# yazinsai/offline-tarteel

Measured on AMD Instinct MI355X. Metric: utterances/sec (10 s @16 kHz), higher is better.
Workload: dtype f16; 1 GPU; c2c-direct-mixed hot path, batch=64/GPU synthetic 10 s/16 kHz clips, FastConformer-CTC forward (fp16 weights) + greedy decode + verse retrieval + CTC rerank (BASELINE.json configs[1]); seeded random weights (real ONNX absent); global_batch=64, parallelism=dp1, gate_failed_utterances_per_batch=64, skip_unused_passes=True, weights=fp16, weights_effective=precision fp16; weights quantised by the engine (none: f16), batches_in_flight=3, concurrent_streams_probe=2

## Files before the change

include/qverse.h:

```cpp
#ifndef QVERSE_H
#define QVERSE_H

#include <stdint.h>

#ifdef __cplusplus
extern "C" {
#endif

#define QV_VOCAB 1025
#define QV_BLANK 1024
#define QV_MAX_TRANSCRIPT 1024
#define QV_MAX_TRANSCRIPT_WIDE 2048

enum {
    QV_OK = 0,
    QV_ERR_ARG = 1,
    QV_ERR_IO = 2,
    QV_ERR_HIP = 3,
    QV_ERR_CAPACITY = 4,
    QV_ERR_NO_MODEL = 5
};

enum { QV_SOURCE_NONE = 0, QV_SOURCE_TEXT = 1, QV_SOURCE_CTC = 2 };

// ... 203 lines not shown
                     qv_align_long_info *info_host, int32_t *first_host, int32_t *last_host, float *logp_host,
                     int32_t pitch, void *stream);
int qv_align_long(qv_engine *e, const float *audio_dev, int64_t audio_pitch, const int64_t *lengths_host, int32_t rows,
                  int32_t window_samples, int32_t margin_frames, const uint16_t *targets_host, const int32_t *lens_host,
                  qv_align_long_info *info_host, int32_t *first_host, int32_t *last_host, float *logp_host,
                  int32_t pitch, void *stream);

#define QV_BEAM_MAX 64
enum { QV_BEAM_COMPLETE = 1 };
typedef struct {
    int32_t node;
    int32_t n_tokens;
    int32_t n_ends;
    int32_t start_verse, span;
    int32_t surah, ayah, ayah_end;
    int32_t below_count;
    int32_t below_verse, below_span;
    int32_t flags;
    double score;
    double blank_score, nonblank_score;
} qv_beam_entry;
typedef struct { int32_t n_entries, t_frames, max_candidates, reserved; } qv_beam_info;

int qv_trie_stats(const char *tables_path, int32_t max_span, int32_t *nodes, int32_t *ends, int32_t *max_depth,
                  int32_t *max_children);
int qv_trie_node_tokens(qv_engine *e, int32_t max_span, int32_t node, int32_t *ids_out, int32_t cap, int32_t *n_out);
int qv_beam_decode(qv_engine *e, const float *logprobs_dev, const int32_t *t_host, int32_t batch, int32_t t_max,
                   int32_t max_span, int32_t beam, int32_t k, qv_beam_info *info_host, qv_beam_entry *entries_host,
                   int32_t *ids_host, int32_t pitch, void *stream);
int qv_beam_batch(qv_engine *e, const float *audio_dev, const int64_t *lengths_host, int32_t batch, int64_t n_max,
                  int32_t max_span, int32_t beam, int32_t k, qv_beam_info *info_host, qv_beam_entry *entries_host,
                  int32_t *ids_host, int32_t pitch, void *stream);

#define QV_SCAN_MAX 32
typedef struct {
    int32_t start_verse, span;
    int32_t surah, ayah, ayah_end;
    int32_t n_tokens;
    float loss, norm;
    double final_score;
} qv_scan_entry;
typedef struct { int32_t n_entries, n_feasible, n_recursions, t_frames; } qv_scan_info;

int qv_scan_stats(const char *tables_path, int32_t t_frames, int32_t max_span, const uint32_t *surah_mask4, int32_t *n_feasible,
                  int32_t *n_recursions, int64_t *state_steps);
int qv_scan_logprobs(qv_engine *e, const float *logprobs_dev, const int32_t *t_host, int32_t batch, int32_t t_max,
                     int32_t max_span, double span_penalty, int32_t k, const uint32_t *surah_mask_host,
                     qv_scan_info *info_host, qv_scan_entry *entries_host, float *loss_out_dev, void *stream);
int qv_scan_batch(qv_engine *e, const float *audio_dev, const int64_t *lengths_host, int32_t batch, int64_t n_max,
                  int32_t max_span, double span_penalty, int32_t k, const uint32_t *surah_mask_host,
                  qv_scan_info *info_host, qv_scan_entry *entries_host, float *loss_out_dev, void *stream);
int qv_scan_kernel_times(qv_engine *e, float *ms2_host);

const int32_t *qv_packed_results_dev(qv_engine *e);


int qv_debug_retrieve(qv_engine *e, const uint8_t *codes_host, int32_t n_codes,
                      int32_t *base_start, int32_t *base_span, double *base_score,
                      int32_t *cand_start, int32_t *cand_span, double *cand_score,
                      int32_t cand_cap, int32_t *n_cand, int32_t *runner_idx, double *runner_score,
                      int32_t *n_runners, void *stream);

int qv_debug_ctc_loss(qv_engine *e, const float *logprobs_dev, int32_t t_frames,
                      const uint16_t *targets_host, const int32_t *lens_host, int32_t n,
                      float *loss_host, void *stream);

int qv_debug_transcript_codes(qv_engine *e, int32_t ctx, int32_t batch, uint8_t *codes_host, int32_t pitch,
                              int32_t *len_host, int32_t *words_host);

int qv_debug_forward_tap(qv_engine *e, int32_t what, int32_t layer, float *out_dev, void *stream);

int qv_profile_gemm(qv_engine *e, int32_t enable);
int qv_profile_gemm_read(qv_engine *e, double *ms21, double *flops21, int32_t *launches21);
int qv_profile_replay_gemm(qv_engine *e, int32_t which, int32_t iters, double *avg_us, double *flops_per_launch,
                           void *stream);
int qv_profile_replay_kernel(qv_engine *e, int32_t which, char *name_out, int32_t name_cap);
int qv_debug_gemm_tiles(int32_t mode);
int qv_debug_gemm_tile_height(int32_t mode);
int qv_debug_gemm_pipeline(int32_t ld, int32_t nst, int32_t narrow);
int qv_debug_attention_variant(int32_t mode);

int qv_debug_kernel_variant(int32_t which, int32_t mode);

int qv_debug_sub01_plan(int64_t n_samples, int32_t batch, int32_t *frames_out, int32_t *run_tiles_out);
int qv_debug_sub35_plan(int64_t n_samples, int32_t batch, int32_t *run_frames_out);

int qv_debug_forward_graph_stats(qv_engine *eng, int64_t *replays, int64_t *captures);
int64_t qv_debug_forward_graph_failures(qv_engine *eng);

int qv_profile_inject_logprobs(qv_engine *e, const float *logprobs_dev, int32_t t_max, const int32_t *t_host, int32_t batch);

int qv_profile_stages(qv_engine *e, int32_t enable);
int qv_stage_times(qv_engine *e, int32_t ctx, float *ms4_host);
int qv_long_kernel_times(qv_engine *e, float *ms3_host);
int qv_align_long_kernel_times(qv_engine *e, float *ms2_host);

int qv_debug_int4_roundtrip(const float *w, int32_t n_rows, int32_t k, float *out);
int qv_debug_int8_roundtrip(const float *w, int32_t n_rows, int32_t k, float *out);

int32_t qv_weight_count(void);
int qv_weight_spec(int32_t index, char *name_out, int32_t name_cap, int32_t *dims4_out, int32_t *ndim_out);
int qv_weight_random(uint64_t seed, int32_t index, float *out, int64_t numel);

int qv_weights_info(qv_engine *e, char *out, int32_t cap);

const char *qv_build_info(void);

#ifdef __cplusplus
}
#endif
#endif
```

offline-tarteel_amd/csrc/qv_capi.hip:

```cpp

#include "qv_common.h"
#include "qv_kernels.h"
#include "qv_layers.h"
#include "qv_long_plan.h"
#include "qv_rows.h"
#include "qv_scan_plan.h"
#include "qv_tables_host.h"
#include "qv_trie_host.h"

#include <math.h>
#include <stdio.h>
#include <string.h>

#include <algorithm>
#include <chrono>
#include <mutex>

static std::string g_create_error;

namespace {
__global__ void k_spin(long long ticks) {
    const long long t0 = wall_clock64();
    while (wall_clock64() - t0 < ticks) __builtin_amdgcn_s_sleep(16);
}
// ... 420 lines not shown
    if (!eng) return QV_ERR_ARG;
    if (enable)
        for (int k = 0; k < eng->n_ctx; ++k)
            for (hipEvent_t &e : eng->ctx[k].stage_ev)
                if (!e) QV_HIP(hipEventCreate(&e));
    eng->profile_stages = enable != 0;
    return QV_OK;
}

extern "C" int qv_stage_times(qv_engine *eng, int32_t k, float *ms4) {
    QV_SERIALISE(eng);
    if (!eng || !ms4 || k < 0 || k >= eng->n_ctx) return QV_ERR_ARG;
    QvCtx &c = eng->ctx[k];
    if (!c.stage_valid) { qv_set_error(eng, "qv_stage_times: no profiled batch on this context (qv_profile_stages first)"); return QV_ERR_ARG; }
    QV_HIP(hipEventSynchronize(c.stage_ev[4]));
    for (int i = 0; i < 4; ++i) QV_HIP(hipEventElapsedTime(&ms4[i], c.stage_ev[i], c.stage_ev[i + 1]));
    return QV_OK;
}

static int fetch_results(qv_engine *eng, QvCtx &c, int batch, int t_max, qv_result *res, int32_t *greedy_host, hipStream_t stream) {
    if (!res || batch < 1 || batch > c.work.max_batch) return QV_ERR_ARG;
    QV_HIP(hipMemcpyAsync(res, c.work.results, sizeof(qv_result) * batch, hipMemcpyDeviceToHost, stream));
    if (greedy_host) {
        int tc = c.work.t_cap;
        int w = t_max < tc ? t_max : tc;
        QV_HIP(hipMemcpy2DAsync(greedy_host, sizeof(int32_t) * t_max, c.work.greedy, sizeof(int32_t) * tc,
                                sizeof(int32_t) * w, batch, hipMemcpyDeviceToHost, stream));
    }
    QV_HIP(hipStreamSynchronize(stream));
    for (int b = 0; b < batch; ++b) {
        if (res[b].source == QV_SOURCE_CTC) res[b].score = exp(-(double)res[b].ctc_norm_loss);
        if (res[b].flags & QV_FLAG_TRANSCRIPT_TRUNCATED) { res[b].surah = res[b].ayah = res[b].ayah_end = 0; }
    }
    return QV_OK;
}

extern "C" int qv_fetch_results(qv_engine *eng, int32_t batch, int32_t t_max, qv_result *res, int32_t *greedy_host,
                                void *stream) {
    QV_SERIALISE(eng);
    if (!eng) return QV_ERR_ARG;
    QV_ORDERED(eng, stream);
    return fetch_results(eng, eng->ctx[eng->cur_ctx], batch, t_max, res, greedy_host, (hipStream_t)stream);
}

extern "C" int qv_decode_retrieve_rerank(qv_engine *eng, const float *lp, const int32_t *t_host, int32_t batch,
                                         int32_t t_max, qv_result *res, int32_t *greedy_host, void *stream) {
    QV_SERIALISE(eng);
    int rc = qv_decode_retrieve_rerank_async(eng, lp, t_host, batch, t_max, stream);
    if (rc) return rc;
    return qv_fetch_results(eng, batch, t_max, res, greedy_host, stream);
}

extern "C" int qv_predict_batch_async(qv_engine *eng, const float *audio_dev, const int64_t *lengths_host,
                                      int32_t batch, int64_t n_max, void *stream) {
    QV_SERIALISE(eng);
    if (!eng) return QV_ERR_ARG;
    QV_TRY(need_model(eng));
    int t_max;
    QV_TRY(batch_in_capacity(eng, "", lengths_host, batch, &t_max));
    QV_ORDERED(eng, stream);
    std::vector<int32_t> t_out(batch);
    hipStream_t run = (hipStream_t)stream;
    if (eng->n_ctx > 1) {
        const int k = eng->next_ctx;
        eng->next_ctx = (k + 1) % eng->n_ctx;
        QvCtx &c = eng->ctx[k];
        if (c.busy) QV_HIP(hipEventSynchronize(c.done));
        eng->cur_ctx = k;
        QV_HIP(hipEventRecord(c.in_ready, (hipStream_t)stream));
        QV_HIP(hipStreamWaitEvent(c.stream, c.in_ready, 0));
        run = c.stream;
    }
    QvCtx &c = eng->ctx[eng->cur_ctx];
    qv_stage_mark(eng, c, 0, run);
    int rc = qv_model_forward(eng, eng->model, eng->cur_ctx, audio_dev, lengths_host, batch, n_max, c.logprobs_ws, t_max,
                              t_out.data(), run, false, eng->n_ctx > 1);
    if (rc) return rc;
    qv_stage_mark(eng, c, 1, run);
    if (eng->inject_lp) {
        if (batch > eng->inject_batch) { qv_set_error(eng, "injected log-probs hold fewer utterances than the batch"); return QV_ERR_ARG; }
        rc = qv_post_run(eng, c, eng->inject_lp, eng->inject_tmax, eng->inject_t.data(), batch, run);
        if (rc == QV_OK) align_note(c, eng->inject_lp, eng->inject_tmax, batch, run);
    } else {
        rc = qv_post_run(eng, c, c.logprobs_ws, t_max, t_out.data(), batch, run);
        if (rc == QV_OK) align_note(c, c.logprobs_ws, t_max, batch, run);
    }
    if (rc) return rc;
    if (eng->n_ctx > 1) {
        QV_HIP(hipEventRecord(c.done, c.stream));
        c.busy = true;
    }
    return QV_OK;
}

extern "C" int qv_predict_batch_async_ctx(qv_engine *eng, const float *audio_dev, const int64_t *lengths_host, int32_t batch,
                                          int64_t n_max, void *stream, int32_t *ctx_out) {
    QV_SERIALISE(eng);
    int rc = qv_predict_batch_async(eng, audio_dev, lengths_host, batch, n_max, stream);
    if (rc == QV_OK && ctx_out) *ctx_out = eng->cur_ctx;
    return rc;
}

extern "C" int qv_predict_batch(qv_engine *eng, const float *audio_dev, const int64_t *lengths_host, int32_t batch,
                                int64_t n_max, qv_result *res, int32_t *greedy_host, void *stream) {
    QV_SERIALISE(eng);
    int rc = qv_predict_batch_async(eng, audio_dev, lengths_host, batch, n_max, stream);
    if (rc) return rc;
    const int last_tmax = eng->ctx[eng->cur_ctx].last_tmax;
    if (eng->n_ctx > 1) return qv_fetch_results_ctx(eng, eng->cur_ctx, batch, last_tmax, res, greedy_host);
    return qv_fetch_results(eng, batch, last_tmax, res, greedy_host, stream);
}

static int fir_for(qv_engine *eng, const float *taps, int32_t n_taps, int32_t up, const qv_engine::Fir **out);

extern "C" int qv_upfirdn(qv_engine *eng, const float *x_dev, int64_t n_in, const float *taps, int32_t n_taps, int32_t up,
                          int32_t down, int64_t m0, int64_t n_out, float *y_dev, void *stream) {
    QV_SERIALISE(eng);
    if (!eng || !x_dev || !taps || !y_dev || n_in < 1 || n_taps < 1 || up < 1 || down < 1 || m0 < 0 || n_out < 0) return QV_ERR_ARG;
    QV_ORDERED(eng, stream);
    const qv_engine::Fir *fir = nullptr;
    QV_TRY(fir_for(eng, taps, n_taps, up, &fir));
    launch_upfirdn(x_dev, n_in, fir->hflip_dev, fir->P, up, down, m0, n_out, y_dev, (hipStream_t)stream);
    QV_HIP(hipGetLastError());
    return QV_OK;
}

static int fir_for(qv_engine *eng, const float *taps, int32_t n_taps, int32_t up, const qv_engine::Fir **out) {
    for (const auto &f : eng->firs)
        if (f.up == up && (int)f.taps.size() == n_taps && memcmp(f.taps.data(), taps, sizeof(float) * n_taps) == 0) { *out = &f; return QV_OK; }
    int P = (n_taps + up - 1) / up;
    std::vector<float> hf((size_t)up * P, 0.f);
    for (int t = 0; t < up; ++t)
        for (int j = 0; j < P; ++j) {
            int k = t + up * (P - 1 - j);
            if (k < n_taps) hf[(size_t)t * P + j] = taps[k];
        }
    float *d = nullptr;
    QV_TRY(qv_dev_zeroed(eng, eng->allocs, hf.size(), &d));
    QV_HIP(hipMemcpy(d, hf.data(), hf.size() * sizeof(float), hipMemcpyHostToDevice));
    eng->firs.push_back({up, std::vector<float>(taps, taps + n_taps), d, P});
    *out = &eng->firs.back();
    return QV_OK;
}

static int resample_slot(qv_engine *eng, unsigned char **slot) {
    if (!eng->resample_tab) QV_TRY(qv_dev_zeroed(eng, eng->allocs, (size_t)QV_RESAMPLE_SLOTS * QV_RESAMPLE_ROWS * 12, &eng->resample_tab));
    *slot = eng->resample_tab + (size_t)(eng->resample_at++ % QV_RESAMPLE_SLOTS) * QV_RESAMPLE_ROWS * 12;
    return QV_OK;
}

extern "C" int qv_upfirdn_batch(qv_engine *eng, const float *x_dev, int64_t x_pitch, const int32_t *src_rows_host,
                                const int64_t *n_in_host, int32_t rows, const float *taps, int32_t n_taps, int32_t up, int32_t down,
                                int64_t m0, float *y_dev, int64_t y_pitch, void *stream) {
    QV_SERIALISE(eng);
    if (!eng || !x_dev || !n_in_host || !taps || !y_dev || rows < 1 || rows > QV_RESAMPLE_ROWS || n_taps < 1 || up < 1 || down < 1 || m0 < 0 ||
        x_pitch < 1 || y_pitch < 1)
        return QV_ERR_ARG;
    for (int r = 0; r < rows; ++r) {
        if (n_in_host[r] < 1 || n_in_host[r] > x_pitch) { qv_set_error(eng, "qv_upfirdn_batch: a row's length is outside [1, x_pitch]"); return QV_ERR_ARG; }
        if ((n_in_host[r] * up + down - 1) / down > y_pitch) { qv_set_error(eng, "qv_upfirdn_batch: y_pitch is shorter than a row's output"); return QV_ERR_ARG; }
        if (src_rows_host && src_rows_host[r] < 0) return QV_ERR_ARG;
    }
    QV_ORDERED(eng, stream);
    const qv_engine::Fir *fir = nullptr;
    QV_TRY(fir_for(eng, taps, n_taps, up, &fir));
    unsigned char *slot = nullptr;
    QV_TRY(resample_slot(eng, &slot));
// ... 540 lines not shown
    memcpy(ms3_host, eng->long_ws.kernel_ms, sizeof(float) * 3);
    return QV_OK;
}

extern "C" int qv_align_long_kernel_times(qv_engine *eng, float *ms2_host) {
    QV_SERIALISE(eng);
    if (!eng || !ms2_host) return QV_ERR_ARG;
    if (!eng->profile_stages || !eng->align_long_ws.big) { qv_set_error(eng, "qv_align_long_kernel_times: no profiled long alignment (qv_profile_stages first)"); return QV_ERR_ARG; }
    memcpy(ms2_host, eng->align_long_ws.kernel_ms, sizeof(float) * 2);
    return QV_OK;
}

extern "C" int qv_debug_forward_tap(qv_engine *eng, int32_t what, int32_t layer, float *out_dev, void *stream) {
    QV_SERIALISE(eng);
    if (!eng) return QV_ERR_ARG;
    if (!eng->model) { qv_set_error(eng, "engine created without a model"); return QV_ERR_NO_MODEL; }
    QV_ORDERED(eng, stream);
    return qv_model_tap(eng, eng->model, eng->cur_ctx, what, layer, out_dev, (hipStream_t)stream);
}

extern "C" int qv_profile_gemm(qv_engine *eng, int32_t enable) {
    if (!eng) return QV_ERR_ARG;
    qv_gemm_prof_enable(enable != 0);
    return QV_OK;
}

extern "C" int qv_profile_gemm_read(qv_engine *eng, double *ms21, double *flops21, int32_t *launches21) {
    if (!eng || !ms21 || !flops21 || !launches21) return QV_ERR_ARG;
    int n[21];
    qv_gemm_prof_collect(ms21, flops21, n);
    for (int i = 0; i < 21; ++i) launches21[i] = n[i];
    return QV_OK;
}

extern "C" int qv_profile_replay_kernel(qv_engine *eng, int32_t which, char *name_out, int32_t name_cap) {
    QV_SERIALISE(eng);
    if (!eng || !name_out || name_cap < 8) return QV_ERR_ARG;
    if (!eng->model) { qv_set_error(eng, "engine created without a model"); return QV_ERR_NO_MODEL; }
    return qv_model_replay_kernel(eng, eng->model, eng->cur_ctx, which, name_out, name_cap);
}

extern "C" int qv_weights_info(qv_engine *eng, char *out, int32_t cap) {
    QV_SERIALISE(eng);
    if (!eng || !out || cap < 16) return QV_ERR_ARG;
    if (!eng->model) { snprintf(out, (size_t)cap, "no acoustic model (post-logits stages only)"); return QV_OK; }
    qv_model_weights_info(eng->model, out, cap);
    return QV_OK;
}

extern "C" int qv_debug_attention_variant(int32_t mode) {
    if (mode < -1 || mode > 5) return QV_ERR_ARG;
    qv_attention_set_variant(mode);
    return QV_OK;
}

extern "C" int qv_debug_kernel_variant(int32_t which, int32_t mode) {
    if (which < 0 || which >= QV_KV_COUNT || mode < -1 || mode > 15) return QV_ERR_ARG;
    qv_kernel_variant_set(which, mode);
    return QV_OK;
}

extern "C" int qv_debug_sub01_plan(int64_t n_samples, int32_t batch, int32_t *frames_out, int32_t *run_tiles_out) {
    if (n_samples < 400 || batch < 1 || !frames_out) return QV_ERR_ARG;
    qv_model_frame_counts(n_samples, frames_out);
    if (run_tiles_out) *run_tiles_out = qv_sub01_run_tiles(batch, frames_out[2], qv_switches_now());
    return QV_OK;
}

extern "C" int qv_debug_sub35_plan(int64_t n_samples, int32_t batch, int32_t *run_frames_out) {
    if (n_samples < 400 || batch < 1 || !run_frames_out) return QV_ERR_ARG;
    int32_t fr[4];
    qv_model_frame_counts(n_samples, fr);
    *run_frames_out = qv_sub35_run_frames(batch, fr[3], qv_switches_now());
    return QV_OK;
}

extern "C" int qv_debug_forward_graph_stats(qv_engine *eng, int64_t *replays, int64_t *captures) {
    QV_SERIALISE(eng);
    if (!eng || !eng->model || !replays || !captures) return QV_ERR_ARG;
    qv_model_graph_stats(eng->model, replays, captures);
    return QV_OK;
}

extern "C" int64_t qv_debug_forward_graph_failures(qv_engine *eng) {
    QV_SERIALISE(eng);
    return (eng && eng->model) ? qv_model_graph_failures(eng->model) : -1;
}

extern "C" int qv_debug_gemm_tiles(int32_t mode) {
    if (mode < -1 || mode > 2) return QV_ERR_ARG;
    qv_gemm_set_t256(mode);
    return QV_OK;
}

extern "C" int qv_debug_gemm_tile_height(int32_t mode) {
    if (mode < -1 || mode > 3) return QV_ERR_ARG;
    qv_gemm_set_bm(mode);
    return QV_OK;
}

extern "C" int qv_debug_gemm_pipeline(int32_t ld, int32_t nst, int32_t narrow) {
    const int ids[3] = {QV_SW_GEMM_LD, QV_SW_GEMM_NST, QV_SW_GEMM_NARROW}, modes[3] = {ld, nst, narrow};
    for (int i = 0; i < 3; ++i)
        if (modes[i] < -1 || modes[i] > QV_SWITCH_TABLE[ids[i]].hi) return QV_ERR_ARG;
    for (int i = 0; i < 3; ++i) qv_switch_set(ids[i], modes[i]);
    return QV_OK;
}

extern "C" int qv_profile_replay_gemm(qv_engine *eng, int32_t which, int32_t iters, double *avg_us, double *flops_per_launch,
                                      void *stream) {
    QV_SERIALISE(eng);
    if (!eng || !avg_us || !flops_per_launch) return QV_ERR_ARG;
    if (!eng->model) { qv_set_error(eng, "engine created without a model"); return QV_ERR_NO_MODEL; }
    return qv_model_replay_gemm(eng, eng->model, eng->cur_ctx, which, iters, avg_us, flops_per_launch, (hipStream_t)stream);
}
```

offline-tarteel_amd/csrc/qv_common.h:

```cpp
#pragma once

#include <hip/hip_runtime.h>
#include <stdint.h>

#include <algorithm>
#include <functional>
#include <mutex>
#include <string>
#include <vector>

#include "../../include/qverse.h"
#include "qv_limits.h"
#include "qv_long_plan.h"
#include "qv_switches.h"

#define QV_CAND_CAP 2048
#define QV_RUNNER_CAP 128
#define QV_RAW_CAP 4096

#define QV_HIP(expr)                                                                         \
    do {                                                                                     \
        hipError_t e_ = (expr);                                                              \
        if (e_ != hipSuccess) {                                                              \
            qv_set_error(eng, std::string(#expr) + ": " + hipGetErrorString(e_));            \
// ... 188 lines not shown
    QvMirror m;
    size_t row_bytes, ops_cap;
    size_t in_off, bp_off;
    size_t bp_row_words;
};
int qv_correct_rows(qv_engine *eng, QvCtx &c, const uint8_t *pred_codes, const int32_t *pred_off, const uint8_t *ref_codes,
                    const int32_t *ref_off, int rows, int flags, qv_correct_info *info_host, uint8_t *ops_host, int ops_pitch,
                    qv_correct_word *words_host, int words_pitch, hipStream_t stream);
int qv_correct_results(qv_engine *eng, int k_ctx, int batch, int flags, qv_correct_info *info_host, uint8_t *ops_host, int ops_pitch,
                       qv_correct_word *words_host, int words_pitch);

int qv_transcribe_rows(qv_engine *eng, QvCtx &c, const float *lp, const int32_t *t_host, int batch, int t_max,
                       qv_transcript_info *info_host, int32_t *ids_host, float *logp_host, int16_t *first_host, int16_t *last_host,
                       int pitch, hipStream_t stream);

struct QvBeamState;
struct QvTrie;
void qv_beam_free(qv_engine *eng);
int qv_beam_trie(qv_engine *eng, int max_span, const QvTrie **out);
int qv_beam_node_tokens(qv_engine *eng, int max_span, int node, int32_t *ids_out, int cap, int32_t *n_out);
int qv_beam_rows(qv_engine *eng, QvCtx &c, const float *lp, const int32_t *t_host, int batch, int t_max, int max_span, int W, int k,
                 qv_beam_info *info_host, qv_beam_entry *entries_host, int32_t *ids_host, int pitch, hipStream_t stream);

struct QvScanState;
void qv_scan_free(qv_engine *eng);
int qv_scan_times(qv_engine *eng, float *ms2);
int qv_scan_rows(qv_engine *eng, QvCtx &c, const float *lp, const int32_t *t_host, int batch, int t_max, int max_span, double penalty,
                 int k, const uint32_t *mask_host, qv_scan_info *info_host, qv_scan_entry *entries_host, float *loss_out_dev,
                 hipStream_t stream);

struct QvLongWs {
    QvMirror m;
    float *batch;
    size_t batch_cap;
    size_t tab_bytes, rec_bytes, out_bytes, fid_bytes;
    float kernel_ms[3];
};
void qv_long_free(QvLongWs &w);
int qv_long_run(qv_engine *eng, QvCtx &c, const float *audio, int64_t audio_pitch, const float *lp_in, int t_max_in,
                const int64_t *n_host, int rows, int window_samples, int margin_frames, qv_long_info *info_host, int32_t *ids_host,
                float *logp_host, int32_t *first_host, int32_t *last_host, int pitch, hipStream_t stream);
struct QvLongWin {
    int64_t src_off;
    int64_t dst;
    int32_t len;
    int32_t lp_win;
    int32_t j0;
    int32_t count;
};
struct QvLongRec { int32_t t_frames, n_windows; };
struct QvLongTimer;
struct QvLongCall {
    std::vector<QvLongPlan> plans;
    std::vector<int64_t> fwd_len;
    size_t n_win;
    int t_top, kw, wn, P;
    const QvLongWin *tab_d;
    const QvLongRec *rec_d;
};
int qv_long_check(qv_engine *eng, const char *who, QvCtx &c, const float *audio, int64_t audio_pitch, int t_max_in,
                  const int64_t *n_host, int rows, int window_samples, int margin_frames, QvLongCall &call);
int qv_long_tables(qv_engine *eng, QvCtx &c, bool audio, int64_t audio_pitch, int rows, QvLongCall &call, hipStream_t stream);
int qv_long_rounds(qv_engine *eng, QvCtx &c, const QvLongCall &call, const float *audio, int64_t audio_pitch, const float *lp_in,
                   int t_max_in, hipStream_t stream, QvLongTimer *tm,
                   const std::function<int(const float *lp, int t_max, size_t k0, int nb)> &per_round);

struct QvAlignLongWs {
    QvMirror m;
    unsigned char *big;
    size_t big_bytes;
    float kernel_ms[3];
};
void qv_align_long_free(QvAlignLongWs &w);
int qv_align_long_run(qv_engine *eng, QvCtx &c, const float *audio, int64_t audio_pitch, const float *lp_in, int t_max_in,
                      const int64_t *n_host, int rows, int window_samples, int margin_frames, const uint16_t *targets_host,
                      const int32_t *lens_host, qv_align_long_info *info_host, int32_t *first_host, int32_t *last_host,
                      float *logp_host, int pitch, hipStream_t stream);

struct QvMatchSet {
    int max_q;
    int decode_threads;
    int frag_blocks;
    size_t trigram_lds;
    void (*k_decode)(QvTables, QvWork, const float *, int, const int32_t *);
    void (*k_prepare_codes)(QvWork, int);
    void (*k_trigram)(QvTables, QvWork), (*k_frag)(QvTables, QvWork);
    void (*k_lcs_full)(QvTables, QvWork, int), (*k_hint_sp)(QvTables, QvWork, int);
    void (*k_spans)(QvTables, QvWork, QvKnobs), (*k_spans2)(QvTables, QvWork, QvKnobs);
    void (*k_track)(QvTables, QvTrack);
    void (*k_ctc_long[2])(QvTables, QvWork, QvKnobs, const float *, int);
};
extern const QvMatchSet qv_match_default __attribute__((visibility("hidden"))), qv_match_wide __attribute__((visibility("hidden")));

int qv_post_tracker_match(qv_engine *eng, const uint8_t *codes_host, const int32_t *offsets_host,
                          const int32_t *n_words_host, const int32_t *bonus_host, int batch,
                          qv_track_match *out_host, hipStream_t stream);
int qv_post_run(qv_engine *eng, QvCtx &c, const float *logprobs_dev, int t_max, const int32_t *t_host, int batch,
                hipStream_t stream);
int qv_post_debug_retrieve(qv_engine *eng, QvCtx &c, const uint8_t *codes_host, int n, hipStream_t stream);
int qv_post_match_verse(qv_engine *eng, QvCtx &c, const uint8_t *codes_host, int n, int n_bonus, const int32_t *bonus_verse,
                        const double *bonus_value, int max_span, hipStream_t stream);
int qv_post_debug_ctc(qv_engine *eng, const float *lp, int T, const uint16_t *tg, const int32_t *lens, int n,
                      float *loss_host, hipStream_t stream);

struct QvModel;
int qv_model_create(qv_engine *eng, const qv_config *cfg, const QvSwitches &sw, QvModel **out);
void qv_model_destroy(QvModel *m);
int qv_model_forward(qv_engine *eng, QvModel *m, int k, const float *audio_dev, const int64_t *len_host, int batch,
                     int64_t n_max, float *logprobs_dev, int t_max, int32_t *t_out_host, hipStream_t stream,
                     bool zero_pad_rows = false,
                     bool may_graph = false);
int qv_model_tap(qv_engine *eng, QvModel *m, int k, int what, int layer, float *out_dev, hipStream_t stream);
void qv_model_frame_counts(int64_t n_samples, int32_t out[4]);
int qv_model_replay_gemm(qv_engine *eng, QvModel *m, int k, int which, int iters, double *avg_us, double *flops, hipStream_t s);
int qv_model_replay_kernel(qv_engine *eng, QvModel *m, int k, int which, char *name_out, int cap);

void qv_model_weights_info(const QvModel *m, char *out, int cap);
void qv_model_graph_stats(const QvModel *m, int64_t *replays, int64_t *captures);
int64_t qv_model_graph_failures(const QvModel *m);
void qv_stage_mark(qv_engine *eng, QvCtx &c, int i, hipStream_t s);

#define QV_MAX_CTX 8
#define QV_STAGE_SLOTS 2
struct QvCtx {
    QvWork work = {};
    float *logprobs_ws = nullptr;
    int32_t *t_host_scratch = nullptr;
    int32_t *t_dev = nullptr;
    hipStream_t stream = nullptr;
    hipEvent_t in_ready = nullptr, done = nullptr;
    bool busy = false;
    int last_batch = 0, last_tmax = 0;
    hipEvent_t t_copied[QV_STAGE_SLOTS] = {};
    bool t_pending[QV_STAGE_SLOTS] = {};
    int t_slot = 0;
    hipEvent_t stage_ev[5] = {};
    bool stage_valid = false;
    struct PostGraph { const float *lp; int batch, t_max, variants; hipGraphExec_t exec; } post_graph[4] = {};
    bool post_graph_off = false;
    int n_post_graph = 0;
    const float *al_lp = nullptr;
    int al_tmax = 0, al_batch = 0;
    hipStream_t al_stream = nullptr;
    std::vector<QvMirror> mirrors;
    QvAlignWs align = {};
    QvNbestWs nbest = {};
    QvCorrectWs correct = {};
    QvRowWs transcribe = {};
    QvRowWs beam = {};
    QvMirror scan = {};
};

struct qv_engine {
    std::recursive_mutex mu;
    hipEvent_t tail_ev = nullptr;
    hipStream_t tail_stream = nullptr;
    bool tail_valid = false;
    qv_config cfg;
    int max_q = QV_MAX_TRANSCRIPT;
    const QvMatchSet *match = &qv_match_default;
    QvKnobs knobs;
    int device;
    std::string last_error;
    QvTables tab;
    std::vector<void *> allocs;
    QvCtx ctx[QV_MAX_CTX];
    int n_ctx, cur_ctx, next_ctx;
    QvModel *model;
    struct Fir { int up; std::vector<float> taps; float *hflip_dev; int P; };
    std::vector<Fir> firs;
    unsigned char *resample_tab = nullptr;
    unsigned resample_at = 0;
    QvTrack track;
    QvLongWs long_ws = {};
    QvAlignLongWs align_long_ws = {};
    QvBeamState *beam = nullptr;
    QvScanState *scan = nullptr;
    bool profile_stages;
    const float *inject_lp;
    int inject_tmax, inject_batch;
    std::vector<int32_t> inject_t;
    std::vector<uint8_t> h_surah;
    std::vector<uint16_t> h_ayah;
};
```

offline-tarteel_amd/csrc/qv_dev_util.h:

```cpp
#pragma once

#include "qv_kernels.h"

static __device__ __forceinline__ float wave_sum(float v) {
#pragma unroll
    for (int o = 32; o > 0; o >>= 1) v += __shfl_xor(v, o);
    return v;
}
static __device__ __forceinline__ float wave_max(float v) {
#pragma unroll
    for (int o = 32; o > 0; o >>= 1) v = fmaxf(v, __shfl_xor(v, o));
    return v;
}
static __device__ __forceinline__ float wave_min(float v) {
#pragma unroll
    for (int o = 32; o > 0; o >>= 1) v = fminf(v, __shfl_xor(v, o));
    return v;
}

static __device__ __forceinline__ int xcd_order(int wg, int nwg) {
    const int q = nwg >> 3, r = nwg & 7, xcd = wg & 7, idx = wg >> 3;
    return (xcd < r ? xcd * (q + 1) : r * (q + 1) + (xcd - r) * q) + idx;
}

static __device__ __forceinline__ void mel_mean_rstd(const double *acc, int b, int f, int tm, float &mean, float &rstd) {
    double s1 = acc[((size_t)b * QV_NMEL + f) * 2], s2 = acc[((size_t)b * QV_NMEL + f) * 2 + 1];
    double mu = s1 / tm, var = (s2 - s1 * mu) / (tm - 1);
    mean = (float)mu;
    rstd = 1.f / (sqrtf((float)(var > 0.0 ? var : 0.0)) + 1e-5f);
}

struct LnParam { f32x4 g0, g1, b0, b1; };
static __device__ __forceinline__ LnParam ln_param(const float *__restrict__ gam, const float *__restrict__ bet, int lane) {
    LnParam p;
    p.g0 = *(const f32x4 *)(gam + lane * 8); p.g1 = *(const f32x4 *)(gam + lane * 8 + 4);
    p.b0 = *(const f32x4 *)(bet + lane * 8); p.b1 = *(const f32x4 *)(bet + lane * 8 + 4);
    return p;
}
static __device__ __forceinline__ void ln_row_p(const float v[8], const LnParam &p, float o[8]) {
    float s = 0.f;
#pragma unroll
    for (int i = 0; i < 8; ++i) s += v[i];
    float mu = wave_sum(s) * (1.f / QV_D);
    float q = 0.f;
#pragma unroll
    for (int i = 0; i < 8; ++i) { float d = v[i] - mu; q += d * d; }
    float rs = rsqrtf(wave_sum(q) * (1.f / QV_D) + 1e-5f);
#pragma unroll
    for (int i = 0; i < 4; ++i) { o[i] = (v[i] - mu) * rs * p.g0[i] + p.b0[i]; o[4 + i] = (v[4 + i] - mu) * rs * p.g1[i] + p.b1[i]; }
}

static __device__ __forceinline__ void conv0_tap_offsets(int hi, int koff[5]) {
#pragma unroll
    for (int j = 0; j < 5; ++j) {
        const int k = 2 * j + hi < 9 ? 2 * j + hi : 8;
        koff[j] = (k / 3) * (QV_NMEL + 2) + k % 3;
    }
}
static __device__ __forceinline__ void conv0_taps(const float *rows, int r0, int f1, const int koff[5], float xb[5]) {
    const float *base = rows + r0 * (QV_NMEL + 2) + 2 * f1;
#pragma unroll
    for (int j = 0; j < 5; ++j) xb[j] = base[koff[j]];
}
```

offline-tarteel_amd/csrc/qv_launch_plan.h:

```cpp
#pragma once

#include "qv_limits.h"
#include "qv_switches.h"

enum GemmWeights { GEMM_W_F16 = 0, GEMM_W_INT4 = 1, GEMM_W_INT8 = 2, GEMM_W_A8W8 = 3 };
struct GemmShape {
    int M, N, K;
    int weights;
    bool has_bias;
    bool glu;
    int in_flight;
};
struct GemmPlan { bool wide, narrow; int nst, bm; };

inline GemmPlan gemm_plan(const GemmShape &g, const QvSwitches &sw) {
    const bool w4 = g.weights == GEMM_W_INT4;
    const int env_nst = sw[QV_SW_GEMM_NST], env_narrow = sw[QV_SW_GEMM_NARROW], env_ld = sw[QV_SW_GEMM_LD];
    GemmPlan p;
    p.narrow = g.N % 128 != 0;
    if (w4 && !p.narrow && (g.N / 128) * ((g.M + 127) / 128) < 400) p.narrow = true;
    if (env_narrow >= 0 && g.N % 128 == 0 && !g.glu) p.narrow = env_narrow != 0;
    const int tiles = (g.N / (p.narrow ? 64 : 128)) * ((g.M + 127) / 128);
    p.nst = tiles >= 400 ? 2 : (g.K / 64 >= 16 ? 4 : 3);
    if (p.narrow && p.nst > 3) p.nst = 3;
    if (env_nst >= 2 && env_nst <= (p.narrow ? 3 : 4)) p.nst = env_nst;
    if (env_ld == 1) p.nst = 0;
    const int t256 = sw[QV_SW_GEMM_T256];
    p.wide = false;
    p.bm = 256;
    if (t256 > 0 && g.N % 256 == 0 && g.has_bias && !(w4 && (g.K % 128 != 0 || g.K > 4096))) {
        const int tiles256 = (g.N / 256) * ((g.M + 255) / 256);
        const int env_min = sw[QV_SW_GEMM_MINTILES], env_min_longk = sw[QV_SW_GEMM_MINTILES_LONGK];
        const bool busy = g.in_flight >= 3;
        const int min_tiles = env_min > 0 ? env_min : g.in_flight >= 4 ? 1 : busy ? 128 : 160;
        const int min_tiles_longk = env_min_longk > 0 ? env_min_longk : busy ? 1 : 160;
        p.wide = t256 >= 2 || tiles256 >= (g.K >= 2048 ? min_tiles_longk : min_tiles);
        const int bm_mode = sw[QV_SW_GEMM_BM];
        if (p.wide && bm_mode > 0) {
            const long tiles192 = (long)(g.N / 256) * ((g.M + 191) / 192);
            const long cost256 = ((tiles256 + 255) / 256) * 256, cost192 = ((tiles192 + 255) / 256) * 192;
            if (bm_mode >= 3 || ((bm_mode == 2 || !busy) && cost192 * 108 <= cost256 * 100)) p.bm = 192;
        }
    }
    return p;
}

struct GemmKernel { int bn, nst, ld; };
inline GemmKernel gemm_kernel(const GemmShape &g, const GemmPlan &p) {
    if (g.weights == GEMM_W_INT8 || g.weights == GEMM_W_A8W8) return {128, 2, 1};
    const int bn = p.narrow && !g.glu ? 64 : 128;
    if (p.nst == 0) return {bn, 2, 1};
    return {bn, p.nst <= 2 ? 2 : p.nst == 3 || bn == 64 ? 3 : 4, 0};
}

inline int sub01_run_tiles(int batch, int t2_max, const QvSwitches &sw) {
    const int n_tiles = (t2_max + SUB_TT - 1) / SUB_TT, forced = sw[QV_KV_SUB_RUN];
    int best = 1;
    if (forced >= 1 && forced <= 4) best = forced == 3 ? SUB_MAX_RUN : forced == 4 ? SUB_RES_RUN : forced;
    else {
        long best_cost = -1;
        for (int run = 1; run <= SUB_RES_RUN; ++run) {
            const long blocks = (long)batch * ((n_tiles + run - 1) / run), cost = (blocks + 511) / 512 * (2 * run + 1);
            if (best_cost < 0 || cost < best_cost) { best = run; best_cost = cost; }
        }
    }
    return best < n_tiles ? best : (n_tiles > 0 ? n_tiles : 1);
}

inline int sub35_run_steps(int batch, int t3_max, const QvSwitches &sw) {
    const int n_steps = (t3_max + S35_TC - 1) / S35_TC, forced = sw[QV_KV_SUB35];
    int best = 1;
    if (forced >= 1 && forced <= 3) best = forced == 3 ? S35_MAX_RUN : forced;
    else {
        long best_cost = -1;
        for (int run = 1; run <= S35_MAX_RUN; ++run) {
            const long blocks = (long)batch * ((n_steps + run - 1) / run), cost = (blocks + 255) / 256 * (run + 1);
            if (best_cost < 0 || cost < best_cost) { best = run; best_cost = cost; }
        }
    }
    return best < n_steps ? best : (n_steps > 0 ? n_steps : 1);
}

enum AttKernel { ATT_NONE, ATT_WS_2_2_192, ATT_WS_1_3_256, ATT_X_192, ATT_OLD };
struct AttentionPlan {
    bool run_short;
    int rest;
    int t_short;
};
inline AttentionPlan attention_plan(int variant, int t_min, int t_max) {
    if (variant == 2) return {false, ATT_OLD, 0};
    AttentionPlan p = {false, ATT_NONE, 0};
    if (variant == 3 || variant == 5) {
        p.t_short = ATT_SHORT_T;
        p.run_short = t_min <= ATT_SHORT_T;
        if (t_max <= ATT_SHORT_T) return p;
    }
    p.rest = variant == 4 || variant == 5 ? ATT_X_192 : variant == 1 ? ATT_WS_1_3_256 : ATT_WS_2_2_192;
    return p;
}
```

offline-tarteel_amd/csrc/qv_layers.h:

```cpp
#pragma once

#include "qv_kernels.h"

struct FrontendTab {
    const float *window;
    const float2 *twiddle;
    const int32_t *mel_lo;
    const int32_t *mel_cnt;
    const float *mel_w;
};

size_t qv_melstats_doubles(size_t max_batch);
void launch_logmel(const float *audio, int64_t n_max, const int32_t *n_samples, const FrontendTab &ft, float *feats,
                   int tm_max, double *stats, int batch, hipStream_t s, const QvSwitches &sw = qv_switches_now());
void launch_melapply(const float *feats, const int32_t *n_samples, int tm_max, const double *stats, float *out, int batch,
                     hipStream_t s);
void launch_conv0(const float *feats, int tm_max, const int32_t *len_in, const double *stats, const float *w,
                  const float *bias, half_t *out, int t1_max, int batch, hipStream_t s);
void launch_sub01(const float *feats, int tm_max, const int32_t *len_mel, const double *stats, const float *w0,
                  const float *b0, const int32_t *len1, const float *w1, const float *b1, half_t *out, int t2_max, int batch,
                  hipStream_t s, const QvSwitches &sw = qv_switches_now());
int qv_sub01_run_tiles(int batch, int t2_max, const QvSwitches &sw = qv_switches_now());
void launch_dwconv2d(const half_t *in, int tin_max, int fin, const int32_t *len_in, const float *w, const float *bias,
                     half_t *out, int tout_max, int fout, int batch, hipStream_t s);
void launch_pack_rows(const half_t *x, int t_max, int row_elems, const int32_t *len, const int32_t *row_off, half_t *y,
                      int32_t *row_map, int batch, hipStream_t s);
void launch_sub35(const half_t *c1, int t2_max, const half_t *w3, const float *b3, const float *w5, const float *b5,
                  const int32_t *len2, const int32_t *len3, const int32_t *row_off, half_t *out, int32_t *row_map, int t3_max,
                  int batch, hipStream_t s, const QvSwitches &sw = qv_switches_now());
void qv_sub35_init();
int qv_sub35_run_frames(int batch, int t3_max, const QvSwitches &sw = qv_switches_now());
void launch_unpack_rows_f32(const half_t *x, int t_max, int row_elems, const int32_t *len, const int32_t *row_off, float *y,
                            int batch, hipStream_t s);
void launch_layernorm(const float *x, const float *g, const float *b, half_t *y, int M, hipStream_t s);
void launch_layernorm2(float *x, const float *g1, const float *b1, const float *g2, const float *b2, half_t *y, int M,
                       hipStream_t s);
void launch_to_half(const float *x, half_t *y, size_t n, hipStream_t s);
void launch_to_float(const half_t *x, float *y, size_t n, hipStream_t s);
void launch_attention(const half_t *qk, const half_t *vt, const half_t *pos, int pos_ld, const float *bu, const float *bv,
                      const int32_t *len, const int32_t *row_off, half_t *out, int t_max, int t_min, int t_pad, int batch,
                      hipStream_t s, const QvSwitches &sw = qv_switches_now());
void launch_dwconv1d(const half_t *x, const float *w, const float *bias, const int32_t *len, const int32_t *row_off, half_t *y,
                     int t_max, int batch, hipStream_t s);
void launch_logsoftmax(const float *logits, int ld, float *out, int M, const int32_t *row_map, int t_out, hipStream_t s);
void launch_zero_pad_rows(float *out, const int32_t *len, int t_out, int t_min, int batch, hipStream_t s);
void launch_upfirdn_rows(const float *x, int64_t x_pitch, const int32_t *src, const int64_t *n_in_rows, int rows, const float *hflip,
                         int P, int up, int down, int64_t m0, float *y, int64_t y_pitch, hipStream_t s);
void launch_mixdown(const float *x, int64_t x_pitch, const int64_t *n_frames, int rows, int channels, float *y, int64_t y_pitch,
                    int64_t max_frames, hipStream_t s);
void launch_upfirdn(const float *x, int64_t n_in, const float *hflip, int P, int up, int down, int64_t m0, int64_t n_out,
                    float *y, hipStream_t s);
```

offline-tarteel_amd/csrc/qv_layers.hip:

```cpp

#include "qv_layers.h"

#include "qv_dev_util.h"
#include "qv_launch_plan.h"
#include "qv_logmel_reg.h"

#include <math.h>

namespace {

__device__ __forceinline__ float sigmoidf_(float x) { return 1.0f / (1.0f + __expf(-x)); }

__global__ __launch_bounds__(256) void k_logmel(const float *__restrict__ audio, int64_t n_max,
                                                const int32_t *__restrict__ n_samples, const FrontendTab ft,
                                                float *__restrict__ feats, int tm_max) {
    __shared__ float2 buf[4][2][256];
    __shared__ float pw[4][264];
    __shared__ float2 tw[256];
    const int wave = threadIdx.x >> 6, lane = threadIdx.x & 63;
    const int b = blockIdx.y, t = blockIdx.x * 4 + wave;
    const int n = n_samples[b];
    const int tm = n / 160 + 1;
    tw[threadIdx.x] = ft.twiddle[threadIdx.x];
    __syncthreads();
// ... 660 lines not shown
            else {
#pragma unroll
                for (int i = 0; i < 8; ++i) o2[i] = o[i];
            }
            half8 h;
#pragma unroll
            for (int i = 0; i < 8; ++i) h[i] = (half_t)o2[i];
            *(half8 *)(y + (size_t)(row0 + r) * QV_D + lane * 8) = h;
        }
    }
}

__global__ void k_to_half(const float *__restrict__ x, half_t *__restrict__ y, size_t n8) {
    size_t i = (size_t)blockIdx.x * blockDim.x + threadIdx.x;
    if (i >= n8) return;
    f32x4 a = *(const f32x4 *)(x + i * 8), c = *(const f32x4 *)(x + i * 8 + 4);
    half8 h = {(half_t)a[0], (half_t)a[1], (half_t)a[2], (half_t)a[3], (half_t)c[0], (half_t)c[1], (half_t)c[2], (half_t)c[3]};
    *(half8 *)(y + i * 8) = h;
}

__global__ void k_to_float(const half_t *__restrict__ x, float *__restrict__ y, size_t n) {
    size_t i = (size_t)blockIdx.x * blockDim.x + threadIdx.x;
    if (i < n) y[i] = (float)x[i];
}

#define DW_TT 4
__global__ __launch_bounds__(256) void k_dwconv1d(const half_t *__restrict__ x, const float *__restrict__ wt ,
                                                  const float *__restrict__ bias, const int32_t *__restrict__ len,
                                                  const int32_t *__restrict__ row_off, half_t *__restrict__ y) {
    const int wg = xcd_order(blockIdx.y * gridDim.x + blockIdx.x, gridDim.x * gridDim.y);
    const int b = wg / gridDim.x, t0 = ((wg - b * gridDim.x) * 4 + (threadIdx.x >> 6)) * DW_TT, lane = threadIdx.x & 63;
    const int T = len[b], c0 = lane * 8;
    if (t0 >= T) return;
    const size_t row0 = (size_t)row_off[b];
    float w[9][8], bs[8];
#pragma unroll
    for (int k = 0; k < 9; ++k) {
        f32x4 w0 = *(const f32x4 *)(wt + k * QV_D + c0), w1 = *(const f32x4 *)(wt + k * QV_D + c0 + 4);
#pragma unroll
        for (int c = 0; c < 4; ++c) { w[k][c] = w0[c]; w[k][4 + c] = w1[c]; }
    }
    {
        f32x4 b0 = *(const f32x4 *)(bias + c0), b1 = *(const f32x4 *)(bias + c0 + 4);
#pragma unroll
        for (int c = 0; c < 4; ++c) { bs[c] = b0[c]; bs[4 + c] = b1[c]; }
    }
    float acc[DW_TT][8];
#pragma unroll
    for (int j = 0; j < DW_TT; ++j)
#pragma unroll
        for (int c = 0; c < 8; ++c) acc[j][c] = bs[c];
#pragma unroll
    for (int i = 0; i < DW_TT + 8; ++i) {
        int tt = t0 - 4 + i;
        if (tt < 0 || tt >= T) continue;
        half8 v = *(const half8 *)(x + (row0 + tt) * QV_D + c0);
        float vf[8];
#pragma unroll
        for (int c = 0; c < 8; ++c) vf[c] = (float)v[c];
#pragma unroll
        for (int j = 0; j < DW_TT; ++j) {
            int k = i - j;
            if (k < 0 || k > 8) continue;
#pragma unroll
            for (int c = 0; c < 8; ++c) acc[j][c] = __builtin_fmaf(w[k][c], vf[c], acc[j][c]);
        }
    }
#pragma unroll
    for (int j = 0; j < DW_TT; ++j) {
        if (t0 + j >= T) break;
        half8 o;
#pragma unroll
        for (int c = 0; c < 8; ++c) o[c] = (half_t)(acc[j][c] * sigmoidf_(acc[j][c]));
        *(half8 *)(y + (row0 + t0 + j) * QV_D + c0) = o;
    }
}

__global__ __launch_bounds__(256) void k_logsoftmax(const float *__restrict__ logits, int ld, float *__restrict__ out, int M,
                                                    const int32_t *__restrict__ row_map, int t_out) {
    int row = blockIdx.x * 4 + (threadIdx.x >> 6), lane = threadIdx.x & 63;
    if (row >= M) return;
    const int bt = row_map[row];
    const size_t orow = (size_t)(bt >> 16) * t_out + (bt & 0xFFFF);
    const float *p = logits + (size_t)row * ld;
    float v[17];
    float mx = -INFINITY;
#pragma unroll
    for (int i = 0; i < 17; ++i) {
        int c = lane + 64 * i;
        v[i] = c < 1025 ? p[c] : -INFINITY;
        mx = fmaxf(mx, v[i]);
    }
    mx = wave_max(mx);
    float s = 0.f;
#pragma unroll
    for (int i = 0; i < 17; ++i) s += (lane + 64 * i < 1025) ? expf(v[i] - mx) : 0.f;
    float lse = mx + logf(wave_sum(s));
    float *o = out + orow * 1025;
#pragma unroll
    for (int i = 0; i < 17; ++i) {
        int c = lane + 64 * i;
        if (c < 1025) o[c] = v[i] - lse;
    }
}

__global__ __launch_bounds__(256) void k_zero_pad_rows(float *__restrict__ out, const int32_t *__restrict__ len, int t_out) {
    const int b = blockIdx.y, t = len[b] + blockIdx.x;
    if (t >= t_out) return;
    float *o = out + ((size_t)b * t_out + t) * 1025;
    for (int c = threadIdx.x; c < 1025; c += 256) o[c] = 0.f;
}

}


size_t qv_melstats_doubles(size_t max_batch) { return max_batch * 2 * QV_NMEL * (1 + MS_CHUNKS); }

void launch_logmel(const float *audio, int64_t n_max, const int32_t *n_samples, const FrontendTab &ft, float *feats,
                   int tm_max, double *stats, int batch, hipStream_t s, const QvSwitches &sw) {
    double *part = stats + (size_t)batch * 2 * QV_NMEL;
    const int variant = sw[QV_KV_LOGMEL];
    if (variant == 2)
        hipLaunchKernelGGL(lmv::k_logmel_run<QV_LOGMEL_RUN>, dim3((tm_max + 4 * QV_LOGMEL_RUN - 1) / (4 * QV_LOGMEL_RUN), batch), dim3(256), 0, s, audio, n_max, n_samples, ft, feats, tm_max);
    else if (variant == 1)
        hipLaunchKernelGGL(lmv::k_logmel_reg<0>, dim3((tm_max + 3) / 4, batch), dim3(256), 0, s, audio, n_max, n_samples, ft, feats, tm_max);
    else
        hipLaunchKernelGGL(k_logmel, dim3((tm_max + 3) / 4, batch), dim3(256), 0, s, audio, n_max, n_samples, ft, feats, tm_max);
    hipLaunchKernelGGL(k_melstats, dim3(MS_CHUNKS, batch), dim3(320), 0, s, feats, n_samples, tm_max, part);
    hipLaunchKernelGGL(k_melstats_sum, dim3(batch), dim3(2 * QV_NMEL), 0, s, part, stats);
}

void launch_melapply(const float *feats, const int32_t *n_samples, int tm_max, const double *stats, float *out, int batch,
                     hipStream_t s) {
    hipLaunchKernelGGL(k_melapply, dim3(64, batch), dim3(320), 0, s, feats, n_samples, tm_max, stats, out);
}

void launch_conv0(const float *feats, int tm_max, const int32_t *len_in, const double *stats, const float *w,
                  const float *bias, half_t *out, int t1_max, int batch, hipStream_t s) {
    hipLaunchKernelGGL(k_conv0, dim3(1, t1_max, batch), dim3(256), 0, s, feats, tm_max, len_in, stats, w, bias, out, t1_max);
}

int qv_sub01_run_tiles(int batch, int t2_max, const QvSwitches &sw) { return sub01_run_tiles(batch, t2_max, sw); }

void launch_sub01(const float *feats, int tm_max, const int32_t *len_mel, const double *stats, const float *w0,
                  const float *b0, const int32_t *len1, const float *w1, const float *b1, half_t *out, int t2_max, int batch,
                  hipStream_t s, const QvSwitches &sw) {
    const int n_tiles = (t2_max + SUB_TT - 1) / SUB_TT, run = sub01_run_tiles(batch, t2_max, sw);
    const dim3 grid(1, (n_tiles + run - 1) / run, batch);
    if (run <= SUB_RES_RUN)
        hipLaunchKernelGGL(k_sub01<true>, grid, dim3(256), 0, s, feats, tm_max, len_mel, stats, w0, b0, len1, w1, b1, out, t2_max, run);
    else
        hipLaunchKernelGGL(k_sub01<false>, grid, dim3(256), 0, s, feats, tm_max, len_mel, stats, w0, b0, len1, w1, b1, out, t2_max, run);
}

void launch_dwconv2d(const half_t *in, int tin_max, int fin, const int32_t *len_in, const float *w, const float *bias,
                     half_t *out, int tout_max, int fout, int batch, hipStream_t s) {
    hipLaunchKernelGGL(k_dwconv2d, dim3(1, (tout_max + DW2_TT - 1) / DW2_TT, batch), dim3(256), 0, s, in, tin_max, fin, len_in, w,
                       bias, out, tout_max, fout);
}

void launch_pack_rows(const half_t *x, int t_max, int row_elems, const int32_t *len, const int32_t *row_off, half_t *y,
                      int32_t *row_map, int batch, hipStream_t s) {
    hipLaunchKernelGGL(k_pack_rows, dim3(1, t_max, batch), dim3(256), 0, s, x, t_max, row_elems, len, row_off, y, row_map);
}

int qv_sub35_run_frames(int batch, int t3_max, const QvSwitches &sw) { return sub35_run_steps(batch, t3_max, sw) * S35_TC; }

void qv_sub35_init() {
    static const int once = [] {
        (void)hipFuncSetAttribute((const void *)k_sub35, hipFuncAttributeMaxDynamicSharedMemorySize, S35_LDS);
        return 0;
    }();
    (void)once;
}

void launch_sub35(const half_t *c1, int t2_max, const half_t *w3, const float *b3, const float *w5, const float *b5,
                  const int32_t *len2, const int32_t *len3, const int32_t *row_off, half_t *out, int32_t *row_map, int t3_max,
                  int batch, hipStream_t s, const QvSwitches &sw) {
    qv_sub35_init();
    const int n_steps = (t3_max + S35_TC - 1) / S35_TC, run = sub35_run_steps(batch, t3_max, sw);
    hipLaunchKernelGGL(k_sub35, dim3(1, (n_steps + run - 1) / run, batch), dim3(512), S35_LDS, s, c1, t2_max, w3, b3, w5, b5, len2,
                       len3, row_off, out, row_map, run);
}

void launch_unpack_rows_f32(const half_t *x, int t_max, int row_elems, const int32_t *len, const int32_t *row_off, float *y,
// ... 172 lines not shown
```

offline-tarteel_amd/csrc/qv_match_body.inc:

```
#define QV_MAXW (QV_MAXQ / 64)

#include "qv_post_util.h"
#include "qv_lcs.h"
#include <type_traits>

namespace QV_MATCH_NS {

#define DEC_WAVES 16
__global__ __launch_bounds__(64 * DEC_WAVES) void k_decode(QvTables tab, QvWork wk, const float *__restrict__ lp, int t_max,
                                                          const int32_t *__restrict__ t_dev) {
    __shared__ uint8_t raw[QV_RAW_CAP];
    __shared__ unsigned long long pm[2][QV_NSYM][QV_MAXW];
    __shared__ int16_t s_fid[QV_FRAME_CAP];
    __shared__ int32_t s_tok[QV_FRAME_CAP];
    const int b = blockIdx.x, tid = threadIdx.x, lane = tid & 63, wave = tid >> 6;
    if (b == 0 && tid == 0) { *wk.n_fail = 0; wk.frag_ctr[0] = 0; wk.frag_ctr[1] = 0; wk.frag_ctr[2] = 0; }
    QvUtt &u = wk.utt[b];
    const int T = t_dev[b];
    for (int t = wave; t < T; t += DEC_WAVES) {
        float best;
        int bi;
        frame_argmax(lp + ((size_t)b * t_max + t) * QV_VOCAB, lane, best, bi);
        if (lane == 0) s_fid[t] = (int16_t)bi;
    }
    __syncthreads();
    if (wave != 0) return;
    int32_t *greedy = wk.greedy + (size_t)b * wk.t_cap;
    int n_tok = 0;
    for (int base = 0; base < T; base += 64) {
        int t = base + lane;
        int id = -1;
        bool keep = false;
        if (t < T) {
            id = s_fid[t];
            int prev = t > 0 ? s_fid[t - 1] : -1;
            keep = id != prev && id != QV_BLANK;
        }
        int tot, r = wave_rank(keep, lane, tot);
        if (keep) { s_tok[n_tok + r] = id; greedy[n_tok + r] = id; }
        n_tok += tot;
    }
    for (int t = n_tok + lane; t < wk.t_cap; t += 64) greedy[t] = -1;
    QV_WSYNC();
    int n_raw = 0;
    bool trunc = false;
    for (int base = 0; base < n_tok; base += 64) {
        int k = base + lane;
        int id = k < n_tok ? s_tok[k] : -1;
        int len = id >= 0 ? (int)(tab.piece_off[id + 1] - tab.piece_off[id]) : 0;
        int incl = len;
#pragma unroll
        for (int o = 1; o < 64; o <<= 1) {
            int x = __shfl_up(incl, o);
            if (lane >= o) incl += x;
        }
        int off = n_raw + incl - len;
        if (off + len > QV_RAW_CAP) { trunc = true; len = 0; }
        const uint8_t *src = tab.piece_codes + (id >= 0 ? tab.piece_off[id] : 0);
        for (int i = 0; i < len; ++i) raw[off + i] = src[i];
        n_raw += __shfl(incl, 63);
    }
    trunc = __any(trunc);
    if (n_raw > QV_RAW_CAP) n_raw = QV_RAW_CAP;
    QV_WSYNC();
    int last_ns = -1;
    for (int i = lane; i < n_raw; i += 64)
        if (raw[i] != 0) last_ns = i;
    last_ns = wave_max_i(last_ns);
    uint8_t *q = wk.q + (size_t)b * QV_MAXQ, *qs = wk.qs + (size_t)b * QV_MAXQ;
    unsigned long long *pmf = &pm[0][0][0];
    for (int i = lane; i < 2 * QV_NSYM * QV_MAXW; i += 64) pmf[i] = 0ull;
    QV_WSYNC();
    int qn = 0, qsn = 0, spaces = 0;
    for (int base = 0; base < n_raw; base += 64) {
        int i = base + lane;
        int c = i < n_raw ? raw[i] : 0;
        bool keep = i < n_raw && (c != 0 ? true : (i > 0 && raw[i - 1] != 0 && i < last_ns));
        int tot, r = wave_rank(keep, lane, tot);
        if (keep && qn + r < QV_MAXQ) {
            q[qn + r] = (uint8_t)c;
            if (c < QV_NSYM) atomicOr(&pm[0][c][(qn + r) >> 6], 1ull << ((qn + r) & 63));
        }
        bool ks = keep && c != 0;
        int tots, rs = wave_rank(ks, lane, tots);
        if (ks && qsn + rs < QV_MAXQ) {
            qs[qsn + rs] = (uint8_t)c;
            if (c < QV_NSYM) atomicOr(&pm[1][c][(qsn + rs) >> 6], 1ull << ((qsn + rs) & 63));
        }
        spaces += tot - tots;
        qn += tot;
        qsn += tots;
    }
    if (qn > QV_MAXQ) trunc = true;
    int flags = 0;
    if (trunc) { flags |= QV_FLAG_TRANSCRIPT_TRUNCATED; qn = 0; qsn = 0; }
    else if (qn == 0) flags |= QV_FLAG_EMPTY_TRANSCRIPT;
    QV_WSYNC();
    uint64_t *gpm = wk.pm + (size_t)b * 2 * QV_NSYM * QV_MAXW;
    for (int i = lane; i < 2 * QV_NSYM * QV_MAXW; i += 64) gpm[i] = trunc ? 0ull : pmf[i];
    if (lane == 0) {
        u.t_frames = T;
        u.n_tok = n_tok;
        u.q_len = qn;
        u.qs_len = qsn;
        u.q_words = qn > 0 ? spaces + 1 : 0;
        u.flags = flags;
// ... 667 lines not shown
```

offline-tarteel_amd/csrc/qv_model.hip:

```cpp

#include "qv_common.h"
#include "qv_graph.h"
#include "qv_layers.h"
#include "qv_ort.h"
#include "qv_model_prep_host.h"

#include <math.h>
#include <stdio.h>
#include <stdlib.h>
#include <string.h>

#include <array>
#include <map>

#define MM_MEL 0
#define MM_C0 1
#define MM_C1 2
#define MM_C1P 3
#define MM_C2 4
#define MM_LAYER(l) (5 + 3 * (l))
#define MM_HEAD (5 + 3 * N_LAYERS)
#define MM_SITES (MM_HEAD + 1)

extern "C" int32_t qv_weight_count(void) { return (int32_t)weight_shapes().size(); }

extern "C" int qv_weight_spec(int32_t index, char *name_out, int32_t name_cap, int32_t *dims4_out, int32_t *ndim_out) {
    static const std::vector<Shape> shapes = weight_shapes();
    if (index < 0 || index >= (int32_t)shapes.size() || !name_out || !dims4_out || !ndim_out) return QV_ERR_ARG;
    const Shape &sh = shapes[index];
    if ((int32_t)sh.name.size() + 1 > name_cap || sh.dims.size() > 4) return QV_ERR_CAPACITY;
    memcpy(name_out, sh.name.c_str(), sh.name.size() + 1);
    *ndim_out = (int32_t)sh.dims.size();
    for (int k = 0; k < 4; ++k) dims4_out[k] = k < (int)sh.dims.size() ? sh.dims[k] : 1;
    return QV_OK;
}

extern "C" int qv_weight_random(uint64_t seed, int32_t index, float *out, int64_t numel) {
    static const std::vector<Shape> shapes = weight_shapes();
    if (index < 0 || index >= (int32_t)shapes.size() || !out) return QV_ERR_ARG;
    std::vector<float> v;
    random_tensor(shapes[index], seed, v);
    if ((int64_t)v.size() != numel) return QV_ERR_ARG;
    memcpy(out, v.data(), sizeof(float) * v.size());
    return QV_OK;
}

#define QV_FWD_GRAPHS 4
struct FwdKey {
    const float *audio; float *logprobs; const half_t *pos; int64_t n_max; int v[9]; QvSwitches sw;
    bool operator==(const FwdKey &o) const {
        return audio == o.audio && logprobs == o.logprobs && pos == o.pos && n_max == o.n_max && !memcmp(v, o.v, sizeof(v)) && sw == o.sw;
    }
};

struct LenRows {
    int32_t *n_samples, *tm, *l1, *l2, *l3, *row_off;
    LenRows(int32_t *base, int max_batch) : n_samples(base), tm(base + max_batch), l1(base + 2 * max_batch), l2(base + 3 * max_batch),
                                            l3(base + 4 * max_batch), row_off(base + 5 * max_batch) {}
    static size_t words(size_t max_batch) { return 6 * max_batch + 1; }
};
struct FwdShape {
    int B, M, T, t_pad;
    int tm_max, t1m, t2m, t3m, t3min;
    int t_max_out, t_min_pad;
};
inline int pad32(int t) { return (t + 31) / 32 * 32; }
using FwdGraphs = FwdGraphCache<FwdKey, hipGraphExec_t, QV_FWD_GRAPHS>;

struct QvActs {
    float *feats, *x, *logits;
    double *mel_stats;
    half_t *c0, *c1, *c1p, *c2, *c2p, *c2k, *ln, *hbuf, *qk, *vt, *att, *glu, *dw, *xh;
    int32_t *lens_dev;
    int32_t *row_map;
    int32_t *lens_host = nullptr;
    hipEvent_t lens_copied[QV_STAGE_SLOTS] = {};
    bool lens_pending[QV_STAGE_SLOTS] = {};
    int lens_slot = 0, lens_last = 0;
    float *tap_x;
    FwdShape last = {};
    bool sub35 = false;
    float *c1f, *c1pf, *c2f, *gluf, *dwf;
    int8_t *q8;
    uint32_t *mm;
    float *tap_lnc, *tap_glu, *tap_dw;
    FwdGraphs fwd_graphs;
};

struct QvModel {
    QvActs ctx_acts[QV_MAX_CTX] = {};
    int n_ctx;
    std::vector<void *> allocs;
    ModelW w;
    bool w4;
    bool ort;
    bool prequant;
    int max_batch, max_samples, tm_cap, t1_cap, t2_cap, t3_cap;
    size_t rows_cap;
    std::map<std::array<int, 4>, half_t *> pos_cache;
    bool save_taps;
    int64_t fwd_replays = 0, fwd_captures = 0, fwd_capture_failures = 0;
};

namespace {

struct DevSink {
    qv_engine *eng;
    QvModel *m;
    template <typename T>
    int operator()(const std::vector<T> &h, const T **dev) { return qv_dev_upload(eng, m->allocs, h.data(), h.size(), dev); }
};

FrontendTab frontend_tab(const ModelW &w) { return {w.window, (const float2 *)w.twiddle, w.mel_lo, w.mel_cnt, w.mel_w}; }

int stage_len(int t) { return (t + 2 - 3) / 2 + 1; }

GemmArgs gemm_args(const half_t *A, const WMat &W, const float *bias, void *out, int M, int N, int K, int ldo, float alpha) {
    GemmArgs g = {};
    g.A = A; g.W = W.w; g.Wq = W.q; g.wscale = W.sc; g.W8 = W.q8; g.w8scale = W.sc8; g.bias = bias; g.out = out;
    g.M = M; g.N = N; g.K = K; g.lda = K; g.ldw = K; g.ldo = ldo; g.alpha = alpha;
    return g;
}
GemmArgs gemm_args(const int8_t *q8, const OrtConv &W, const float *bias, void *out, int M, int N, int K, int ldo,
                   const RowOwner &own, const uint32_t *mm_in, uint32_t *mm_out) {
    GemmArgs g = {};
    g.A = (const half_t *)q8; g.Wi8 = W.wq; g.wsum = W.wsum; g.w_scale = W.scale; g.bias = bias; g.out = out;
    g.M = M; g.N = N; g.K = K; g.lda = K; g.ldw = K; g.ldo = ldo; g.alpha = 1.f;
    g.row_map = own.row_map; g.len = own.len; g.rows_per_utt = own.rows_per_utt; g.f_per_t = own.f_per_t;
    g.mm_in = mm_in; g.mm_out = mm_out;
    return g;
}

int get_pos(qv_engine *eng, QvModel *m, int t_max, const QvSwitches &sw, hipStream_t stream, const half_t **out) {
    const std::array<int, 4> key = {t_max, sw[QV_SW_GEMM_LD], sw[QV_SW_GEMM_NST], sw[QV_SW_GEMM_NARROW]};
    auto it = m->pos_cache.find(key);
    if (it != m->pos_cache.end()) { *out = it->second; return QV_OK; }
    int R = 2 * t_max - 1;
    std::vector<half_t> pe((size_t)R * QV_D);
    for (int r = 0; r < R; ++r) {
        float pos = (float)(t_max - 1 - r);
        for (int i = 0; i < QV_D / 2; ++i) {
            float div = expf((float)(2 * i) * -(logf(10000.0f) / (float)QV_D));
            pe[(size_t)r * QV_D + 2 * i] = (half_t)sinf(pos * div);
            pe[(size_t)r * QV_D + 2 * i + 1] = (half_t)cosf(pos * div);
        }
    }
    half_t *d_pe = nullptr, *d_out = nullptr;
    QV_HIP(hipMalloc((void **)&d_pe, pe.size() * sizeof(half_t)));
    QV_HIP(hipMalloc((void **)&d_out, (size_t)R * N_LAYERS * QV_D * sizeof(half_t)));
    QV_HIP(hipMemcpyAsync(d_pe, pe.data(), pe.size() * sizeof(half_t), hipMemcpyHostToDevice, stream));
    launch_gemm(EPI_F16, gemm_args(d_pe, m->w.pos_w, m->w.zero_bias, d_out, R, N_LAYERS * QV_D, QV_D, N_LAYERS * QV_D, 1.f), stream, sw);
    QV_HIP(hipStreamSynchronize(stream));
    QV_HIP(hipFree(d_pe));
    m->allocs.push_back(d_out);
    m->pos_cache[key] = d_out;
    *out = d_out;
    return QV_OK;
}

int alloc_context(qv_engine *eng, QvModel *m, int k, bool sub_unfused, bool sub35_unfused) {
    QvActs &a = m->ctx_acts[k];
    const size_t Bz = (size_t)m->max_batch, M = m->rows_cap, lens_words = LenRows::words(Bz);
    TRY(qv_dev_zeroed(eng, m->allocs, Bz * m->tm_cap * QV_NMEL, &a.feats));
    TRY(qv_dev_zeroed(eng, m->allocs, qv_melstats_doubles(Bz), &a.mel_stats));
    if (sub_unfused) TRY(qv_dev_zeroed(eng, m->allocs, Bz * m->t1_cap * 40 * QV_SUBC, &a.c0));
    TRY(qv_dev_zeroed(eng, m->allocs, Bz * m->t2_cap * 20 * QV_SUBC, &a.c1));
    a.sub35 = !m->ort && !sub35_unfused;
    if (!a.sub35) TRY(qv_dev_zeroed(eng, m->allocs, Bz * m->t2_cap * 20 * QV_SUBC, &a.c1p));
    TRY(qv_dev_zeroed(eng, m->allocs, Bz * m->t3_cap * 10 * QV_SUBC, &a.c2));
    if (!a.sub35) TRY(qv_dev_zeroed(eng, m->allocs, Bz * m->t3_cap * 10 * QV_SUBC, &a.c2p));
    TRY(qv_dev_zeroed(eng, m->allocs, Bz * m->t3_cap * 10 * QV_SUBC, &a.c2k));
    TRY(qv_dev_zeroed(eng, m->allocs, M * QV_D, &a.x));
    TRY(qv_dev_zeroed(eng, m->allocs, M * QV_D, &a.ln));
    TRY(qv_dev_zeroed(eng, m->allocs, M * QV_FF, &a.hbuf));
    TRY(qv_dev_zeroed(eng, m->allocs, M * 2 * QV_D, &a.qk));
    TRY(qv_dev_zeroed(eng, m->allocs, Bz * QV_D * pad32(m->t3_cap), &a.vt));
    TRY(qv_dev_zeroed(eng, m->allocs, M * QV_D, &a.att));
    TRY(qv_dev_zeroed(eng, m->allocs, M * QV_D, &a.glu));
    TRY(qv_dev_zeroed(eng, m->allocs, M * QV_D, &a.dw));
    TRY(qv_dev_zeroed(eng, m->allocs, M * QV_D, &a.xh));
    TRY(qv_dev_zeroed(eng, m->allocs, M * HEAD_N, &a.logits));
    TRY(qv_dev_zeroed(eng, m->allocs, lens_words, &a.lens_dev));
    TRY(qv_dev_zeroed(eng, m->allocs, M, &a.row_map));
    QV_HIP(hipHostMalloc((void **)&a.lens_host, sizeof(int32_t) * lens_words * QV_STAGE_SLOTS, hipHostMallocDefault));
    for (int i = 0; i < QV_STAGE_SLOTS; ++i) QV_HIP(hipEventCreateWithFlags(&a.lens_copied[i], hipEventDisableTiming));
    if (m->save_taps) TRY(qv_dev_zeroed(eng, m->allocs, (size_t)(N_LAYERS + 1) * M * QV_D, &a.tap_x));
    if (m->ort) {
        TRY(qv_dev_zeroed(eng, m->allocs, Bz * m->t2_cap * 20 * QV_SUBC, &a.c1f));
        TRY(qv_dev_zeroed(eng, m->allocs, Bz * m->t2_cap * 20 * QV_SUBC, &a.c1pf));
        TRY(qv_dev_zeroed(eng, m->allocs, Bz * m->t3_cap * 10 * QV_SUBC, &a.c2f));
        TRY(qv_dev_zeroed(eng, m->allocs, M * QV_D, &a.gluf));
        TRY(qv_dev_zeroed(eng, m->allocs, M * QV_D, &a.dwf));
        TRY(qv_dev_zeroed(eng, m->allocs, std::max(Bz * m->t2_cap * 20 * QV_SUBC, M * QV_D), &a.q8));
        TRY(qv_dev_zeroed(eng, m->allocs, (size_t)MM_SITES * Bz * QV_MM_STRIDE, &a.mm));
        if (m->save_taps) {
            TRY(qv_dev_zeroed(eng, m->allocs, (size_t)N_LAYERS * M * QV_D, &a.tap_lnc));
            TRY(qv_dev_zeroed(eng, m->allocs, (size_t)N_LAYERS * M * QV_D, &a.tap_glu));
            TRY(qv_dev_zeroed(eng, m->allocs, (size_t)N_LAYERS * M * QV_D, &a.tap_dw));
        }
    }
    return QV_OK;
}

}

int qv_model_create(qv_engine *eng, const qv_config *cfg, const QvSwitches &sw, QvModel **out) {
    if (cfg->precision != QV_PREC_FP16 && cfg->precision != QV_PREC_MIXED_INT4_INT8 && cfg->precision != QV_PREC_ORT_MIXED) {
        qv_set_error(eng, "unknown precision (QV_PREC_FP16, QV_PREC_MIXED_INT4_INT8 or QV_PREC_ORT_MIXED)");
        return QV_ERR_ARG;
    }
    QvModel *m = new QvModel();
    *out = m;
    m->ort = cfg->precision == QV_PREC_ORT_MIXED;
    m->w4 = cfg->precision == QV_PREC_MIXED_INT4_INT8 || m->ort;
    HostWeights hw;
    if (cfg->weights_path && cfg->weights_path[0]) {
        std::string err;
        if (int rc = load_weight_file(cfg->weights_path, hw, err)) { qv_set_error(eng, err); return rc; }
    } else init_random(hw, cfg->random_weights_seed);
    m->prequant = hw.prequantised();
    {
        DevSink sink = {eng, m};
        std::string err;
        WeightPrep<DevSink> prep = {sink, m->w4, m->ort, m->prequant, m->w, err};
        int rc = prep.build_frontend();
        try {
            if (!rc) rc = prep.prepare_weights(hw);
        } catch (const QvMissingWeight &e) {
            qv_set_error(eng, e.what());
            return QV_ERR_IO;
        }
        if (rc && !err.empty()) qv_set_error(eng, err);
        if (rc) return rc;
    }
    int B = cfg->max_batch;
    m->max_batch = B;
    m->max_samples = cfg->max_samples;
    m->tm_cap = cfg->max_samples / 160 + 1;
    m->t1_cap = stage_len(m->tm_cap);
    m->t2_cap = stage_len(m->t1_cap);
    m->t3_cap = stage_len(m->t2_cap);
    const size_t Bz = (size_t)B, M = m->rows_cap = Bz * m->t3_cap;
    {
        const size_t worst = std::max(std::max(Bz * m->t2_cap * 20 * QV_SUBC * 2, M * 2560 * 2), std::max(M * QV_FF * 2, M * HEAD_N * 4));
        if (worst >= (1ull << 31)) {
            qv_set_error(eng, "max_batch x max_samples too large: a GEMM operand would exceed the 2 GiB one buffer descriptor addresses "
                              "(reduce max_batch or max_samples; e.g. 256 x 30 s fits, 2048 x 10 s does not -- shard across engines)");
            return QV_ERR_CAPACITY;
        }
    }
    m->save_taps = sw[QV_SW_DEBUG_TAPS] != 0;
    m->n_ctx = eng->n_ctx;
    qv_sub35_init();
    for (int k = 0; k < m->n_ctx; ++k) TRY(alloc_context(eng, m, k, sw[QV_SW_SUB_UNFUSED] != 0, sw[QV_SW_SUB35_UNFUSED] != 0));
    return QV_OK;
}

void qv_model_destroy(QvModel *m) {
    if (!m) return;
    for (void *p : m->allocs) (void)hipFree(p);
    for (QvActs &a : m->ctx_acts) {
        for (int i = 0; i < a.fwd_graphs.n; ++i) (void)hipGraphExecDestroy(a.fwd_graphs.slot[i].handle);
        if (a.lens_host) (void)hipHostFree(a.lens_host);
        for (hipEvent_t e : a.lens_copied) if (e) (void)hipEventDestroy(e);
    }
    delete m;
}

namespace {

LenRows dev_lens(const QvModel *m, const QvActs &a) { return {a.lens_dev, m->max_batch}; }
LenRows host_lens(const QvModel *m, const QvActs &a, int slot) { return {a.lens_host + slot * LenRows::words(m->max_batch), m->max_batch}; }

int fwd_shape(qv_engine *eng, const QvModel *m, QvActs &a, const int64_t *len_host, int batch, int64_t n_max, int t_max_out,
              bool zero_pad_rows, int32_t *t_out_host, hipStream_t s, FwdShape *out) {
    if (batch < 1 || batch > m->max_batch) { qv_set_error(eng, "batch exceeds engine capacity"); return QV_ERR_CAPACITY; }
    FwdShape sh = {};
    sh.B = batch; sh.t3min = INT32_MAX; sh.t_max_out = t_max_out;
    const int slot = a.lens_slot;
    if (a.lens_pending[slot]) { QV_HIP(hipEventSynchronize(a.lens_copied[slot])); a.lens_pending[slot] = false; }
    const LenRows lh = host_lens(m, a, slot);
    for (int b = 0; b < batch; ++b) {
        int64_t n = len_host[b];
        if (n < 400 || n > n_max || n > m->max_samples) {
            qv_set_error(eng, "utterance length out of range (need 400 <= n <= capacity)");
            return QV_ERR_CAPACITY;
        }
        int tm = (int)(n / 160 + 1), l1 = stage_len(tm), l2 = stage_len(l1), l3 = stage_len(l2);
        lh.n_samples[b] = (int32_t)n; lh.tm[b] = tm; lh.l1[b] = l1; lh.l2[b] = l2; lh.l3[b] = l3;
        sh.tm_max = std::max(sh.tm_max, tm); sh.t1m = std::max(sh.t1m, l1); sh.t2m = std::max(sh.t2m, l2); sh.t3m = std::max(sh.t3m, l3);
        sh.t3min = std::min(sh.t3min, l3);
        t_out_host[b] = l3;
        lh.row_off[b] = sh.M;
        sh.M += l3;
    }
    lh.row_off[batch] = sh.M;
    if (t_max_out < sh.t3m) { qv_set_error(eng, "t_max smaller than the longest utterance's frame count"); return QV_ERR_ARG; }
    sh.T = sh.t3m; sh.t_pad = pad32(sh.T); sh.t_min_pad = zero_pad_rows ? std::min(t_max_out, sh.t3min) : -1;
    QV_HIP(hipMemcpyAsync(a.lens_dev, lh.n_samples, sizeof(int32_t) * LenRows::words(m->max_batch), hipMemcpyHostToDevice, s));
    QV_HIP(hipEventRecord(a.lens_copied[slot], s));
    a.lens_pending[slot] = true;
    a.lens_last = slot;
    a.lens_slot = (slot + 1) % QV_STAGE_SLOTS;
    *out = sh;
    return QV_OK;
}

#ifdef QV_DEV_HOOKS
int hook_skip() { return qv_switches_env()[QV_SW_SKIP]; }
int hook_dup() { return qv_switches_env()[QV_SW_DUP]; }
#else
constexpr int hook_skip() { return 0; }
constexpr int hook_dup() { return 0; }
#endif
template <typename Fn>
inline void hooked(int bit, Fn &&launch, bool may_dup = true) {
    if (!(hook_skip() & bit)) launch();
    if (may_dup && (hook_dup() & bit)) launch();
}

GemmArgs layer_gemm_args(const QvModel *m, const QvActs &a, int M, int T, const half_t *A, int K, const WMat &W, const float *bias,
                         void *out, int N, int ldo, float alpha) {
    GemmArgs g = gemm_args(A, W, bias, out, M, N, K, ldo, alpha);
    g.out2 = a.vt; g.t_max = T; g.t_pad = pad32(T); g.row_map = a.row_map; g.in_flight = m->n_ctx;
    return g;
}
GemmArgs ort_pw1_args(const QvModel *m, const QvActs &a, int M, int l) {
    uint32_t *mm_ln = a.mm + (size_t)MM_LAYER(l) * m->max_batch * QV_MM_STRIDE;
    return gemm_args(a.q8, m->w.L[l].o_pw1, m->w.L[l].pw1_b, a.gluf, M, 2 * QV_D, QV_D / 2, QV_D, RowOwner{a.row_map, nullptr, 0, 0}, mm_ln,
                     mm_ln + (size_t)m->max_batch * QV_MM_STRIDE);
}

struct Fwd {
    qv_engine *eng; const QvModel *m; const QvActs &a; const FwdShape &sh; const LenRows d; const float *audio; int64_t n_max;
    const half_t *posp; const QvSwitches &sw; hipStream_t s;
    uint32_t *mm(int site) const { return a.mm + (size_t)site * m->max_batch * QV_MM_STRIDE; }
// ... 17 lines not shown
        if (a.sub35) {
            launch_sub35(a.c1, sh.t2m, m->w.pw3_w, m->w.pw3_b, m->w.dw5_w, m->w.dw5_b, d.l2, d.l3, d.row_off, a.c2, a.row_map, sh.t3m, sh.B, s, sw);
            pw(a.c2, m->w.pw6_w, m->w.pw6_b, a.c2k, sh.M * 10);
        } else {
            pw(a.c1, m->w.pw3_w, m->w.pw3_b, a.c1p, sh.B * sh.t2m * 20);
            launch_dwconv2d(a.c1p, sh.t2m, 20, d.l2, m->w.dw5_w, m->w.dw5_b, a.c2, sh.t3m, 10, sh.B, s);
            pw(a.c2, m->w.pw6_w, m->w.pw6_b, a.c2p, sh.B * sh.t3m * 10);
            launch_pack_rows(a.c2p, sh.t3m, 10 * QV_SUBC, d.l3, d.row_off, a.c2k, a.row_map, sh.B, s);
        }
        sub_out();
    }
    void frontend_ort() const {
        const int B = sh.B, M2 = B * sh.t2m * 20, M3 = B * sh.t3m * 10;
        const RowOwner own2 = {nullptr, d.l2, sh.t2m * 20, 20}, own3 = {nullptr, d.l3, sh.t3m * 10, 10};
        launch_mm_init(a.mm, (size_t)MM_SITES * m->max_batch * QV_MM_STRIDE, s);
        launch_logmel(audio, n_max, d.n_samples, frontend_tab(m->w), a.feats, sh.tm_max, a.mel_stats, B, s, sw);
        launch_mel_minmax(a.feats, d.n_samples, sh.tm_max, a.mel_stats, mm(MM_MEL), B, s);
        for (int pass = 0; pass < 2; ++pass)
            launch_sub01_ort(pass, a.feats, sh.tm_max, d.tm, a.mel_stats, m->w.o_c0.wq, m->w.o_c0.scale, m->w.c0_b, d.l1, m->w.o_dw2.wq,
                             m->w.o_dw2.scale, m->w.dw2_b, d.l2, mm(MM_MEL), mm(MM_C0), mm(MM_C1), a.c1f, sh.t2m, B, s, sw);
        launch_quant_rows(a.c1f, M2, QV_SUBC, own2, mm(MM_C1), a.q8, s);
        launch_gemm(EPI_F32_RELU, gemm_args(a.q8, m->w.o_pw3, m->w.pw3_b, a.c1pf, M2, QV_SUBC, QV_SUBC / 2, QV_SUBC, own2, mm(MM_C1), mm(MM_C1P)), s, sw);
        launch_dwconv2d_ort(a.c1pf, sh.t2m, 20, d.l2, m->w.o_dw5.wq, m->w.o_dw5.scale, m->w.dw5_b, d.l3, mm(MM_C1P), mm(MM_C2), a.c2f, sh.t3m, 10, B, s);
        launch_quant_rows(a.c2f, M3, QV_SUBC, own3, mm(MM_C2), a.q8, s);
        launch_gemm(EPI_F16_RELU, gemm_args(a.q8, m->w.o_pw6, m->w.pw6_b, a.c2p, M3, QV_SUBC, QV_SUBC / 2, QV_SUBC, own3, mm(MM_C2), nullptr), s, sw);
        launch_pack_rows(a.c2p, sh.t3m, 10 * QV_SUBC, d.l3, d.row_off, a.c2k, a.row_map, B, s);
        sub_out();
    }
    void gemm(int epi, const half_t *A, int K, const WMat &W, const float *bias, void *out, int N, int ldo, float alpha) const {
        const GemmArgs g = layer_gemm_args(m, a, sh.M, sh.T, A, K, W, bias, out, N, ldo, alpha);
        hooked(64, [&] { launch_gemm(epi, g, s, sw); }, epi != EPI_RESID);
    }
    void layernorm(const LayerW &L, int i, bool may_dup = true) const {
        hooked(1, [&] { launch_layernorm(a.x, L.ln_g[i], L.ln_b[i], a.ln, sh.M, s); }, may_dup);
    }
    void ffn_half(const WMat &w1, const float *b1, const WMat &w2, const float *b2) const {
        gemm(EPI_F16_SWISH, a.ln, QV_D, w1, b1, a.hbuf, QV_FF, QV_FF, 1.f);
        gemm(EPI_RESID, a.hbuf, QV_FF, w2, b2, a.x, QV_D, QV_D, 0.5f);
    }
    void attention_block(const LayerW &L, int l) const {
        layernorm(L, 1);
        gemm(EPI_QKV, a.ln, QV_D, L.qkv_w, L.qkv_b, a.qk, 3 * QV_D, 2 * QV_D, 1.f);
        hooked(4, [&] {
            launch_attention(a.qk, a.vt, posp + (size_t)l * QV_D, N_LAYERS * QV_D, L.bias_u, L.bias_v, d.l3, d.row_off, a.att, sh.T, sh.t3min,
                             sh.t_pad, sh.B, s, sw);
        });
        gemm(EPI_RESID, a.att, QV_D, L.out_w, L.out_b, a.x, QV_D, QV_D, 1.f);
    }
    void conv_module_f16(const LayerW &L) const {
        layernorm(L, 2);
        gemm(EPI_GLU, a.ln, QV_D, L.pw1_w, L.pw1_b, a.glu, 2 * QV_D, QV_D, 1.f);
        hooked(8, [&] { launch_dwconv1d(a.glu, L.dw_w, L.dw_b, d.l3, d.row_off, a.dw, sh.T, sh.B, s); });
        gemm(EPI_RESID, a.dw, QV_D, L.pw2_w, L.pw2_b, a.x, QV_D, QV_D, 1.f);
    }
    int conv_module_ort(const LayerW &L, int l) const {
        uint32_t *mm_ln = mm(MM_LAYER(l)), *mm_glu = mm(MM_LAYER(l) + 1), *mm_dw = mm(MM_LAYER(l) + 2);
        const RowOwner own = {a.row_map, nullptr, 0, 0};
        const size_t n = (size_t)sh.M * QV_D, tap_off = l * n;
        launch_ln_minmax(a.x, L.ln_g[2], L.ln_b[2], sh.M, a.row_map, mm_ln, m->save_taps ? a.tap_lnc + tap_off : nullptr, s);
        launch_ln_quant(a.x, L.ln_g[2], L.ln_b[2], sh.M, a.row_map, mm_ln, a.q8, s);
        launch_gemm(EPI_GLU, ort_pw1_args(m, a, sh.M, l), s, sw);
        launch_dwconv1d_ort(a.gluf, L.o_dw.wq, L.o_dw.scale, L.o_dw_b, L.bn_alpha, L.bn_beta, d.l3, d.row_off, mm_glu, mm_dw, a.dwf, sh.T, sh.B, s);
        launch_quant_rows(a.dwf, sh.M, QV_D, own, mm_dw, a.q8, s);
        launch_gemm(EPI_RESID, gemm_args(a.q8, L.o_pw2, L.pw2_b, a.x, sh.M, QV_D, QV_D / 2, QV_D, own, mm_dw, nullptr), s, sw);
        if (m->save_taps) {
            QV_HIP(hipMemcpyAsync(a.tap_glu + tap_off, a.gluf, sizeof(float) * n, hipMemcpyDeviceToDevice, s));
            QV_HIP(hipMemcpyAsync(a.tap_dw + tap_off, a.dwf, sizeof(float) * n, hipMemcpyDeviceToDevice, s));
        }
        return QV_OK;
    }
    int save_x(int idx) const {
        const size_t n = (size_t)sh.M * QV_D;
        if (m->save_taps) QV_HIP(hipMemcpyAsync(a.tap_x + idx * n, a.x, sizeof(float) * n, hipMemcpyDeviceToDevice, s));
        return QV_OK;
    }
    int layer_out(int l) const {
        const LayerW &L = m->w.L[l];
        hooked(2, [&] {
            if (l + 1 < N_LAYERS) launch_layernorm2(a.x, L.ln_g[4], L.ln_b[4], m->w.L[l + 1].ln_g[0], m->w.L[l + 1].ln_b[0], a.ln, sh.M, s);
            else launch_layernorm2(a.x, L.ln_g[4], L.ln_b[4], nullptr, nullptr, a.xh, sh.M, s);
        }, false);
        return save_x(l + 1);
    }
    void ctc_head() const {
        if (m->ort) {
            const RowOwner own = {a.row_map, nullptr, 0, 0};
            launch_rows_minmax(a.x, sh.M, a.row_map, mm(MM_HEAD), s);
            launch_quant_rows(a.x, sh.M, QV_D, own, mm(MM_HEAD), a.q8, s);
            launch_gemm(EPI_F32, gemm_args(a.q8, m->w.o_head, m->w.head_b, a.logits, sh.M, HEAD_N, QV_D / 2, HEAD_N, own, mm(MM_HEAD), nullptr), s, sw);
        } else {
            launch_gemm(EPI_F32, gemm_args(a.xh, WMat{m->w.head_w}, m->w.head_b, a.logits, sh.M, HEAD_N, QV_D, HEAD_N, 1.f), s, sw);
        }
    }
};

int launch_all(qv_engine *eng, const QvModel *m, const QvActs &a, const FwdShape &sh, const float *audio, int64_t n_max, float *logprobs,
               const half_t *posp, const QvSwitches &sw, hipStream_t s) {
    const Fwd f = {eng, m, a, sh, dev_lens(m, a), audio, n_max, posp, sw, s};
    if (m->ort) f.frontend_ort();
    else if (!(hook_skip() & 32)) f.frontend_f16();
    else
        launch_pack_rows(a.sub35 ? a.c2 : a.c2p, sh.t3m, 10 * QV_SUBC, f.d.l3, f.d.row_off, a.c2k, a.row_map, sh.B, s);
    TRY(f.save_x(0));
    f.layernorm(m->w.L[0], 0, false);
    for (int l = 0; l < N_LAYERS; ++l) {
        const LayerW &L = m->w.L[l];
        f.ffn_half(L.ff1_w1, L.ff1_b1, L.ff1_w2, L.ff1_b2);
        f.attention_block(L, l);
        if (m->ort) TRY(f.conv_module_ort(L, l));
        else f.conv_module_f16(L);
        f.layernorm(L, 3);
        f.ffn_half(L.ff2_w1, L.ff2_b1, L.ff2_w2, L.ff2_b2);
        TRY(f.layer_out(l));
    }
    if (hook_skip() & 2) launch_to_half(a.x, a.xh, (size_t)sh.M * QV_D, s);
    f.ctc_head();
    launch_logsoftmax(a.logits, HEAD_N, logprobs, sh.M, a.row_map, sh.t_max_out, s);
    if (sh.t_min_pad >= 0) launch_zero_pad_rows(logprobs, f.d.l3, sh.t_max_out, sh.t_min_pad, sh.B, s);
    return QV_OK;
}

FwdKey fwd_key(const FwdShape &sh, const float *audio, float *logprobs, const half_t *posp, int64_t n_max, const QvSwitches &sw) {
    return {audio, logprobs, posp, n_max, {sh.B, sh.M, sh.T, sh.t3min, sh.tm_max, sh.t1m, sh.t2m, sh.t_max_out, sh.t_min_pad}, sw.forward_part()};
}

}

int qv_model_forward(qv_engine *eng, QvModel *m, int k, const float *audio, const int64_t *len_host, int batch, int64_t n_max,
                     float *logprobs, int t_max_out, int32_t *t_out_host, hipStream_t s, bool zero_pad_rows, bool may_graph) {
    QvActs &a = m->ctx_acts[k];
    FwdShape sh;
    TRY(fwd_shape(eng, m, a, len_host, batch, n_max, t_max_out, zero_pad_rows, t_out_host, s, &sh));
    const QvSwitches sw = qv_switches_now();
    const half_t *posp = nullptr;
    TRY(get_pos(eng, m, sh.T, sw, s, &posp));
    auto plain = [&] { return launch_all(eng, m, a, sh, audio, n_max, logprobs, posp, sw, s); };
    FwdGraphs &graphs = a.fwd_graphs;
    FwdGraphs::Plan plan = {graphs.PLAIN, -1, false};
    if (sw[QV_KV_FWD_GRAPH] == 1 && may_graph && !m->save_taps && !eng->profile_stages && !qv_gemm_prof_on()) {
        const FwdKey key = fwd_key(sh, audio, logprobs, posp, n_max, sw);
        plan = graphs.next(key);
        if (plan.act == graphs.CAPTURE) {
            hipGraphExec_t exec = nullptr;
            bool captured = false;
            TRY(qv_capture_graph(s, plain, &exec, &captured));
            if (captured) {
                if (plan.evict) {
                    QV_HIP(hipStreamSynchronize(s));
                    (void)hipGraphExecDestroy(graphs.slot[plan.slot].handle);
                }
                graphs.store(plan.slot, key, exec);
                m->fwd_captures++;
                plan.act = graphs.REPLAY;
            } else {
                graphs.disabled = true;
                m->fwd_capture_failures++;
                plan.act = graphs.PLAIN;
            }
        }
    }
    if (plan.act == graphs.REPLAY) { QV_HIP(hipGraphLaunch(graphs.slot[plan.slot].handle, s)); m->fwd_replays++; }
    else TRY(plain());
    QV_HIP(hipGetLastError());
    a.last = sh;
    return QV_OK;
}

static int replay_args(qv_engine *eng, QvModel *m, int k, int which, GemmArgs &g, int &epi) {
    QvActs &a = m->ctx_acts[k];
    const int M = a.last.M, T = a.last.T;
    if (M <= 0) { qv_set_error(eng, "replay needs a previous forward"); return QV_ERR_ARG; }
    const LayerW &L = m->w.L[0];
    auto args = [&](const half_t *A, int K, const WMat &W, const float *bias, void *out, int N, int ldo, float alpha) {
        return layer_gemm_args(m, a, M, T, A, K, W, bias, out, N, ldo, alpha);
    };
    switch (which) {
        case 0: epi = EPI_F16_SWISH; g = args(a.ln, QV_D, L.ff1_w1, L.ff1_b1, a.hbuf, QV_FF, QV_FF, 1.f); break;
        case 1: epi = EPI_RESID; g = args(a.hbuf, QV_FF, L.ff1_w2, L.ff1_b2, a.x, QV_D, QV_D, 0.f); break;
        case 2: epi = EPI_QKV; g = args(a.ln, QV_D, L.qkv_w, L.qkv_b, a.qk, 3 * QV_D, 2 * QV_D, 1.f); break;
        case 3: epi = EPI_RESID; g = args(a.att, QV_D, L.out_w, L.out_b, a.x, QV_D, QV_D, 0.f); break;
        case 4: epi = EPI_GLU; g = args(a.ln, QV_D, L.pw1_w, L.pw1_b, a.glu, 2 * QV_D, QV_D, 1.f); break;
        default: return QV_ERR_ARG;
    }
    if (which == 4 && m->ort) {
        const GemmArgs f16 = g;
        g = ort_pw1_args(m, a, M, 0);
        g.out2 = f16.out2; g.t_max = f16.t_max; g.t_pad = f16.t_pad; g.in_flight = f16.in_flight;
    }
    return QV_OK;
}

void qv_model_graph_stats(const QvModel *m, int64_t *replays, int64_t *captures) {
    *replays = m->fwd_replays;
    *captures = m->fwd_captures;
}
int64_t qv_model_graph_failures(const QvModel *m) { return m->fwd_capture_failures; }

void qv_model_weights_info(const QvModel *m, char *out, int cap) {
    const char *prec = m->ort ? "ort-mixed" : m->w4 ? "mixed-int4-int8" : "fp16";
    if (!m->prequant)
        snprintf(out, (size_t)cap, "precision %s; weights quantised by the engine%s", prec, m->w4 ? " (symmetric block-128 int4 Linear)" : " (none: f16)");
    else
        snprintf(out, (size_t)cap, "precision %s; pre-quantised file: %d Linear tensors on the file's own int4 grid (W4A16), %d as "
                 "dequantised f16 values%s", prec, m->w.prequant_w4_linears, m->w.prequant_f16_linears,
                 m->ort ? "; Conv weights on the file's int8 integers" : m->w4 ? "; pointwise-conv weights as dequantised f16 values" : "");
}

int qv_model_replay_kernel(qv_engine *eng, QvModel *m, int k, int which, char *name_out, int cap) {
    GemmArgs g;
    int epi = 0;
    int rc = replay_args(eng, m, k, which, g, epi);
    if (rc != QV_OK) return rc;
    snprintf(name_out, (size_t)cap, "%s", qv_gemm_kernel_name(epi, g, qv_switches_now()));
    return QV_OK;
}

int qv_model_replay_gemm(qv_engine *eng, QvModel *m, int k, int which, int iters, double *avg_us, double *flops, hipStream_t s) {
    if (iters < 1) return QV_ERR_ARG;
    const QvSwitches sw = qv_switches_now();
    GemmArgs g;
    int epi = 0;
    int rc = replay_args(eng, m, k, which, g, epi);
    if (rc != QV_OK) return rc;
    hipEvent_t e0, e1;
    QV_HIP(hipEventCreate(&e0));
    QV_HIP(hipEventCreate(&e1));
    for (int i = 0; i < 3; ++i) launch_gemm(epi, g, s, sw);
    QV_HIP(hipEventRecord(e0, s));
    for (int i = 0; i < iters; ++i) launch_gemm(epi, g, s, sw);
    QV_HIP(hipEventRecord(e1, s));
    QV_HIP(hipEventSynchronize(e1));
    float ms = 0.f;
    QV_HIP(hipEventElapsedTime(&ms, e0, e1));
    (void)hipEventDestroy(e0);
    (void)hipEventDestroy(e1);
    *avg_us = (double)ms * 1e3 / iters;
    *flops = 2.0 * (double)g.M * (double)g.N * (double)g.K * (g.Wi8 ? 2.0 : 1.0);
    return QV_OK;
}

void qv_model_frame_counts(int64_t n_samples, int32_t out[4]) {
    out[0] = (int32_t)(n_samples / 160 + 1);
    for (int i = 1; i < 4; ++i) out[i] = stage_len(out[i - 1]);
}

enum Tap {
    TAP_MEL_NORM = 0, TAP_SUB_OUT = 1, TAP_LAYER_OUT = 2, TAP_ORT_LNC = 3, TAP_ORT_GLU = 4, TAP_ORT_DW = 5, TAP_ORT_C1 = 6,
    TAP_ORT_C1P = 7, TAP_ORT_C2 = 8, TAP_ORT_C2P = 9, TAP_LOGMEL = 10, TAP_C1 = 11, TAP_C2 = 12
// ... 56 lines not shown
```

offline-tarteel_amd/csrc/qv_postlogits.hip:

```cpp

#include "qv_common.h"
#include "qv_graph.h"
#include "qv_greedy.h"
#include "qv_kernels.h"
#include "qv_post_util.h"

#include <math.h>

#include <algorithm>

namespace {

__global__ void k_set_hint(QvWork wk, int b, int n, int v0, int v1, int v2, double b0, double b1, double b2) {
    QvUtt &u = wk.utt[b];
    u.force_full = 1;
    u.hint_n = n;
    u.hint_v[0] = v0; u.hint_v[1] = v1; u.hint_v[2] = v2;
    u.hint_bonus[0] = b0; u.hint_bonus[1] = b1; u.hint_bonus[2] = b2;
    u.hint_sp[0] = u.hint_sp[1] = u.hint_sp[2] = 0.0;
}

__global__ __launch_bounds__(256) void k_pass1_final(QvTables tab, QvWork wk, QvKnobs kn) {
    extern __shared__ __attribute__((aligned(16))) unsigned char smem[];
    double *sc = (double *)smem;
// ... 372 lines not shown
            float norm = __fdiv_rn(wk.cand_loss[(size_t)b * QV_CAND_CAP + c], (float)L);
            r.source = QV_SOURCE_CTC;
            r.ctc_norm_loss = norm;
            r.score = exp(-(double)norm);
            r.surah = tab.surah[st]; r.ayah = tab.ayah[st]; r.ayah_end = r.ayah + sp - 1;
            u.win = c; u.win_norm = norm;
        } else if (u.base_start >= 0) {
            r.source = QV_SOURCE_TEXT;
            r.score = u.base_score;
            r.surah = tab.surah[u.base_start]; r.ayah = tab.ayah[u.base_start];
            r.ayah_end = r.ayah + u.base_span - 1;
        }
    }
    wk.results[b] = r;
    wk.packed[b * 4 + 0] = r.surah;
    wk.packed[b * 4 + 1] = r.ayah;
    wk.packed[b * 4 + 2] = r.ayah_end;
    wk.packed[b * 4 + 3] = __float_as_int((float)r.score);
}

__global__ void k_init_utts(QvWork wk, const int32_t *__restrict__ t_dev, int batch) {
    int b = blockIdx.x * blockDim.x + threadIdx.x;
    if (b == 0) { *wk.n_fail = 0; wk.frag_ctr[0] = 0; wk.frag_ctr[1] = 0; wk.frag_ctr[2] = 0; }
    if (b < batch) wk.utt[b].t_frames = t_dev[b];
}

__global__ void k_track_final(QvTables tab, QvTrack tw, int batch, int nblk) {
    int b = blockIdx.x * blockDim.x + threadIdx.x;
    if (b >= batch) return;
    double best = 0.0;
    unsigned long long key = ~0ull;
    for (int i = 0; i < nblk; ++i) {
        double s = tw.part_s[(size_t)b * QV_TRACK_BLOCKS + i];
        unsigned long long k = tw.part_k[(size_t)b * QV_TRACK_BLOCKS + i];
        if (better(s, k, best, key)) { best = s; key = k; }
    }
    qv_track_match r;
    r.verse = -1; r.surah = 0; r.ayah = 0; r.variant = 0; r.n_words = 0; r.reserved = 0; r.score = 0.0;
    if (best > 0.0 && key != ~0ull) {
        int v = (int)(key >> 1), nb = (int)(key & 1ull);
        r.verse = v; r.surah = tab.surah[v]; r.ayah = tab.ayah[v];
        r.variant = nb ? 2 : 0; r.n_words = tab.nw[nb ? 2 : 0][v]; r.score = best;
    }
    tw.out[b] = r;
}

}


static size_t select_lds(const QvTables &tab) { return (size_t)tab.n_verses * 8 + 128 * 8 + 128 * 4 + 272 * 4 + 128 * 4 + 128 * 8 + 64; }

static void launch_match(const QvMatchSet &set, const QvTables &tab, const QvWork &wk, const QvKnobs &kn, int batch, int lcs_y,
                         bool hint, int force_ctc, hipStream_t stream, const QvSwitches &sw) {
    hipLaunchKernelGGL(set.k_trigram, dim3(batch), dim3(256), (size_t)tab.n_verses * 8 + set.trigram_lds, stream, tab, wk);
    hipLaunchKernelGGL(set.k_lcs_full, dim3(batch, lcs_y), dim3(256), 0, stream, tab, wk, 0);
    hipLaunchKernelGGL(set.k_frag, dim3(set.frag_blocks), dim3(256), 0, stream, tab, wk);
    if (hint) hipLaunchKernelGGL(set.k_hint_sp, dim3(1), dim3(64), 0, stream, tab, wk, 0);
    hipLaunchKernelGGL(k_pass1_final, dim3(batch), dim3(256), select_lds(tab), stream, tab, wk, kn);
    auto k_span_pass = sw[QV_KV_SPANS] == 1 ? set.k_spans2 : set.k_spans;
    hipLaunchKernelGGL(k_span_pass, dim3(QV_SPAN_BLOCKS, batch), dim3(256), 0, stream, tab, wk, kn);
    hipLaunchKernelGGL(k_base_final, dim3((batch + 63) / 64), dim3(64), 0, stream, tab, wk, kn, batch, force_ctc);
}

static void launch_retrieval(qv_engine *eng, QvCtx &c, int batch, int force_ctc, hipStream_t stream, const QvSwitches &sw) {
    const QvMatchSet &set = *eng->match;
    const QvTables &tab = eng->tab;
    const QvWork &wk = c.work;
    const QvKnobs &kn = eng->knobs;
    launch_match(set, tab, wk, kn, batch, 32, false, force_ctc, stream, sw);
    hipLaunchKernelGGL(set.k_lcs_full, dim3(batch, 74), dim3(256), 0, stream, tab, wk, 1);
    hipLaunchKernelGGL(set.k_frag, dim3(set.frag_blocks), dim3(256), 0, stream, tab, wk);
    hipLaunchKernelGGL(k_topk, dim3(batch, 2), dim3(256), select_lds(tab), stream, tab, wk, kn);
    hipLaunchKernelGGL(k_candidates, dim3(batch), dim3(256), (size_t)CAND_PCAP * 12 + CAND_HT * 8 + 1200, stream, tab, wk, kn);
}

static void launch_ctc(const QvMatchSet &set, bool long_targets, int variant, const QvTables &tab, const QvWork &wk, const QvKnobs &kn,
                       const float *lp, int t_max, int batch, hipStream_t stream) {
    const int v = variant != 0;
    auto k = v ? k_ctc<false, 1> : k_ctc<false, 0>;
    if (long_targets) k = set.k_ctc_long[v] ? set.k_ctc_long[v] : (v ? k_ctc<true, 1> : k_ctc<true, 0>);
    hipLaunchKernelGGL(k, dim3(batch, 64), dim3(256), 0, stream, tab, wk, kn, lp, t_max);
}

int qv_post_run(qv_engine *eng, QvCtx &c, const float *lp, int t_max, const int32_t *t_host, int batch, hipStream_t stream) {
    const QvSwitches sw = qv_switches_now();
    const QvMatchSet &set = *eng->match;
    QvTables &tab = eng->tab;
    QvWork &wk = c.work;
    if (batch > wk.max_batch || t_max > wk.t_cap) {
        qv_set_error(eng, "batch or frame count exceeds engine capacity");
        return QV_ERR_CAPACITY;
    }
    for (int b = 0; b < batch; ++b)
        if (t_host[b] < 0 || t_host[b] > t_max) { qv_set_error(eng, "t_host[b] out of range"); return QV_ERR_ARG; }
    {
        const int slot = c.t_slot;
        c.t_slot = (slot + 1) % QV_STAGE_SLOTS;
        if (c.t_pending[slot]) { QV_HIP(hipEventSynchronize(c.t_copied[slot])); c.t_pending[slot] = false; }
        int32_t *th = c.t_host_scratch + (size_t)slot * wk.max_batch;
        for (int b = 0; b < batch; ++b) th[b] = t_host[b];
        QV_HIP(hipMemcpyAsync(c.t_dev, th, sizeof(int32_t) * batch, hipMemcpyHostToDevice, stream));
        QV_HIP(hipEventRecord(c.t_copied[slot], stream));
        c.t_pending[slot] = true;
    }
#ifdef QV_DEV_HOOKS
    const int skip = sw[QV_SW_SKIP];
#else
    constexpr int skip = 0;
#endif
    auto launch_chain = [&]() -> int {
        if (skip & 128) return QV_OK;
        hipLaunchKernelGGL(set.k_decode, dim3(batch), dim3(set.decode_threads), 0, stream, tab, wk, lp, t_max, c.t_dev);
        qv_stage_mark(eng, c, 2, stream);
        launch_retrieval(eng, c, batch, 0, stream, sw);
        qv_stage_mark(eng, c, 3, stream);
        if (!(skip & 16)) launch_ctc(set, t_max > 384, sw[QV_KV_CTC], tab, wk, eng->knobs, lp, t_max, batch, stream);
        hipLaunchKernelGGL(k_result, dim3(batch), dim3(256), 0, stream, tab, wk, batch);
        qv_stage_mark(eng, c, 4, stream);
        return QV_OK;
    };
    QvCtx::PostGraph *hit = nullptr;
    if (sw[QV_SW_POST_GRAPH] != 0 && !c.post_graph_off && eng->n_ctx > 1 && stream == c.stream && lp == c.logprobs_ws && !eng->profile_stages) {
        const int variants = sw[QV_KV_SPANS] | (sw[QV_KV_CTC] << 4) | ((set.max_q > QV_MAX_TRANSCRIPT) << 8);
        for (int i = 0; i < c.n_post_graph; ++i)
            if (c.post_graph[i].lp == lp && c.post_graph[i].batch == batch && c.post_graph[i].t_max == t_max && c.post_graph[i].variants == variants)
                hit = &c.post_graph[i];
        if (!hit && c.n_post_graph < 4) {
            hipGraphExec_t exec = nullptr;
            bool captured = false;
            int rc = qv_capture_graph(stream, launch_chain, &exec, &captured);
            if (rc) return rc;
            if (captured) {
                c.post_graph[c.n_post_graph] = {lp, batch, t_max, variants, exec};
                hit = &c.post_graph[c.n_post_graph++];
            } else c.post_graph_off = true;
        }
    }
    if (hit) QV_HIP(hipGraphLaunch(hit->exec, stream));
    else {
        int rc = launch_chain();
        if (rc) return rc;
    }
    QV_HIP(hipGetLastError());
    c.last_batch = batch;
    c.last_tmax = t_max;
    return QV_OK;
}

static int upload_codes(qv_engine *eng, QvCtx &c, const uint8_t *codes_host, int n, hipStream_t stream) {
    static const int32_t zero = 0;
    QV_HIP(hipMemcpyAsync(c.t_dev, &zero, sizeof(int32_t), hipMemcpyHostToDevice, stream));
    hipLaunchKernelGGL(k_init_utts, dim3(1), dim3(64), 0, stream, c.work, c.t_dev, 1);
    if (n > 0) QV_HIP(hipMemcpyAsync(c.work.q, codes_host, n, hipMemcpyHostToDevice, stream));
    hipLaunchKernelGGL(eng->match->k_prepare_codes, dim3(1), dim3(64), 0, stream, c.work, n);
    return QV_OK;
}

int qv_post_debug_retrieve(qv_engine *eng, QvCtx &c, const uint8_t *codes_host, int n, hipStream_t stream) {
    const QvSwitches sw = qv_switches_now();
    if (n > eng->match->max_q) { qv_set_error(eng, "transcript longer than the engine's max_transcript"); return QV_ERR_CAPACITY; }
    int rc = upload_codes(eng, c, codes_host, n, stream);
    if (rc) return rc;
    launch_retrieval(eng, c, 1, 1, stream, sw);
    QV_HIP(hipGetLastError());
    QV_HIP(hipStreamSynchronize(stream));
    return QV_OK;
}

int qv_post_debug_ctc(qv_engine *eng, const float *lp, int T, const uint16_t *tg, const int32_t *lens, int n,
                      float *loss_host, hipStream_t stream) {
    const QvSwitches sw = qv_switches_now();
    std::vector<int32_t> off(n + 1, 0);
    for (int i = 0; i < n; ++i) {
        if (lens[i] <= 0 || 2 * lens[i] + 1 > 768) { qv_set_error(eng, "target length unsupported"); return QV_ERR_ARG; }
        off[i + 1] = off[i] + lens[i];
    }
    uint16_t *d_t = nullptr;
    int32_t *d_o = nullptr;
    float *d_l = nullptr;
    QV_HIP(hipMalloc(&d_t, sizeof(uint16_t) * std::max(1, off[n])));
    QV_HIP(hipMalloc(&d_o, sizeof(int32_t) * (n + 1)));
    QV_HIP(hipMalloc(&d_l, sizeof(float) * std::max(1, n)));
    QV_HIP(hipMemcpyAsync(d_t, tg, sizeof(uint16_t) * off[n], hipMemcpyHostToDevice, stream));
    QV_HIP(hipMemcpyAsync(d_o, off.data(), sizeof(int32_t) * (n + 1), hipMemcpyHostToDevice, stream));
    if (sw[QV_KV_CTC] == 0) hipLaunchKernelGGL(k_ctc_debug<0>, dim3(n), dim3(64), 0, stream, lp, T, d_t, d_o, n, d_l);
    else hipLaunchKernelGGL(k_ctc_debug<1>, dim3(n), dim3(64), 0, stream, lp, T, d_t, d_o, n, d_l);
    QV_HIP(hipMemcpyAsync(loss_host, d_l, sizeof(float) * n, hipMemcpyDeviceToHost, stream));
    QV_HIP(hipStreamSynchronize(stream));
    (void)hipFree(d_t); (void)hipFree(d_o); (void)hipFree(d_l);
    return QV_OK;
}

int qv_post_tracker_match(qv_engine *eng, const uint8_t *codes_host, const int32_t *offsets_host,
                          const int32_t *n_words_host, const int32_t *bonus_host, int batch,
                          qv_track_match *out_host, hipStream_t stream) {
    QvTrack &tw = eng->track;
    const int nblk = (eng->tab.n_verses + 255) / 256;
    if (nblk > QV_TRACK_BLOCKS) { qv_set_error(eng, "verse table larger than the tracker workspace"); return QV_ERR_CAPACITY; }
    std::vector<int32_t> meta((size_t)QV_TRACK_CAP * 4);
    for (int b0 = 0; b0 < batch; b0 += QV_TRACK_CAP) {
        int nb = std::min(QV_TRACK_CAP, batch - b0);
        const int32_t base = offsets_host[b0];
        for (int i = 0; i < nb; ++i) {
            meta[i * 4] = offsets_host[b0 + i + 1] - offsets_host[b0 + i];
            meta[i * 4 + 1] = n_words_host[b0 + i];
            meta[i * 4 + 2] = bonus_host[b0 + i];
            meta[i * 4 + 3] = offsets_host[b0 + i] - base;
        }
        const int32_t total = offsets_host[b0 + nb] - base;
        if (total > 0) QV_HIP(hipMemcpyAsync(tw.q, codes_host + base, (size_t)total, hipMemcpyHostToDevice, stream));
        QV_HIP(hipMemcpyAsync(tw.meta, meta.data(), sizeof(int32_t) * 4 * nb, hipMemcpyHostToDevice, stream));
        hipLaunchKernelGGL(eng->match->k_track, dim3(nb, nblk), dim3(256), 0, stream, eng->tab, tw);
        hipLaunchKernelGGL(k_track_final, dim3((nb + 63) / 64), dim3(64), 0, stream, eng->tab, tw, nb, nblk);
        QV_HIP(hipGetLastError());
        QV_HIP(hipMemcpyAsync(out_host + b0, tw.out, sizeof(qv_track_match) * nb, hipMemcpyDeviceToHost, stream));
        QV_HIP(hipStreamSynchronize(stream));
    }
    return QV_OK;
}

int qv_post_match_verse(qv_engine *eng, QvCtx &c, const uint8_t *codes_host, int n, int n_bonus, const int32_t *bonus_verse,
                        const double *bonus_value, int max_span, hipStream_t stream) {
    const QvSwitches sw = qv_switches_now();
    QvKnobs kn = eng->knobs;
    kn.max_span = max_span;
    int rc = upload_codes(eng, c, codes_host, n, stream);
// ... 11 lines not shown
```

offline-tarteel_amd/csrc/qv_switches.h:

```cpp
#pragma once

#include <stdlib.h>

#include <atomic>
#include <initializer_list>

enum {
    QV_KV_LOGMEL = 0, QV_KV_ORT_SUB = 1, QV_KV_SPANS = 2, QV_KV_FWD_GRAPH = 3, QV_KV_CTC = 4, QV_KV_SUB_RUN = 5, QV_KV_SUB35 = 6,
    QV_KV_RESERVED = 7, QV_KV_COUNT = 8,
    QV_SW_ATT = 8, QV_SW_ATT_OLD, QV_SW_ATT_HPB, QV_SW_ATT_TILED, QV_SW_ATT_X,
    QV_SW_GEMM_T256, QV_SW_GEMM_BM, QV_SW_GEMM_NST, QV_SW_GEMM_NARROW, QV_SW_GEMM_LD, QV_SW_GEMM_MINTILES, QV_SW_GEMM_MINTILES_LONGK,
    QV_SW_DEBUG_TAPS, QV_SW_SUB_UNFUSED, QV_SW_SUB35_UNFUSED, QV_SW_POST_GRAPH, QV_SW_CU_PARTITION,
#ifdef QV_DEV_HOOKS
    QV_SW_SKIP, QV_SW_DUP,
#endif
    QV_SW_COUNT
};

enum QvParse {
    QV_PARSE_NONE,
    QV_PARSE_DIGIT,
    QV_PARSE_ATOI,
    QV_PARSE_ONE
};

enum QvWhen { QV_READ_ONCE, QV_READ_AT_CREATE };

struct QvSwitchRow { int id; const char *env; int dflt, lo, hi; QvParse parse; QvWhen when; };

inline constexpr QvSwitchRow QV_SWITCH_TABLE[QV_SW_COUNT] = {
    {QV_KV_LOGMEL, "QVERSE_LOGMEL", 2, 0, 15, QV_PARSE_DIGIT, QV_READ_ONCE},
    {QV_KV_ORT_SUB, "QVERSE_ORT_SUB", 1, 0, 15, QV_PARSE_DIGIT, QV_READ_ONCE},
    {QV_KV_SPANS, "QVERSE_SPANS", 1, 0, 15, QV_PARSE_DIGIT, QV_READ_ONCE},
    {QV_KV_FWD_GRAPH, "QVERSE_FWD_GRAPH", 1, 0, 15, QV_PARSE_DIGIT, QV_READ_ONCE},
    {QV_KV_CTC, "QVERSE_CTC", 1, 0, 15, QV_PARSE_DIGIT, QV_READ_ONCE},
    {QV_KV_SUB_RUN, "QVERSE_SUB_RUN", 0, 0, 15, QV_PARSE_DIGIT, QV_READ_ONCE},
    {QV_KV_SUB35, nullptr, 0, 0, 15, QV_PARSE_NONE, QV_READ_ONCE},
    {QV_KV_RESERVED, nullptr, 0, 0, 15, QV_PARSE_NONE, QV_READ_ONCE},
    {QV_SW_ATT, nullptr, 3, 0, 5, QV_PARSE_NONE, QV_READ_ONCE},
    {QV_SW_ATT_OLD, "QVERSE_ATT_OLD", 0, 0, 1, QV_PARSE_ONE, QV_READ_ONCE},
    {QV_SW_ATT_HPB, "QVERSE_ATT_HPB", 0, 0, 1, QV_PARSE_ONE, QV_READ_ONCE},
    {QV_SW_ATT_TILED, "QVERSE_ATT_TILED", 0, 0, 1, QV_PARSE_ONE, QV_READ_ONCE},
    {QV_SW_ATT_X, "QVERSE_ATT_X", 0, 0, 1, QV_PARSE_ONE, QV_READ_ONCE},
    {QV_SW_GEMM_T256, "QVERSE_GEMM_T256", 1, 0, 2, QV_PARSE_ATOI, QV_READ_ONCE},
    {QV_SW_GEMM_BM, "QVERSE_GEMM_BM", 1, 0, 3, QV_PARSE_ATOI, QV_READ_ONCE},
    {QV_SW_GEMM_NST, "QVERSE_GEMM_NST", 0, 0, 4, QV_PARSE_ATOI, QV_READ_ONCE},
    {QV_SW_GEMM_NARROW, "QVERSE_GEMM_NARROW", -1, -1, 1, QV_PARSE_ATOI, QV_READ_ONCE},
    {QV_SW_GEMM_LD, "QVERSE_GEMM_LD", 1, 0, 1, QV_PARSE_ATOI, QV_READ_ONCE},
    {QV_SW_GEMM_MINTILES, "QVERSE_GEMM_MINTILES", 0, 0, 1 << 30, QV_PARSE_ATOI, QV_READ_ONCE},
    {QV_SW_GEMM_MINTILES_LONGK, "QVERSE_GEMM_MINTILES_LONGK", 0, 0, 1 << 30, QV_PARSE_ATOI, QV_READ_ONCE},
    {QV_SW_DEBUG_TAPS, "QVERSE_DEBUG_TAPS", 0, 0, 1, QV_PARSE_ONE, QV_READ_AT_CREATE},
    {QV_SW_SUB_UNFUSED, "QVERSE_SUB_UNFUSED", 0, 0, 1, QV_PARSE_ONE, QV_READ_AT_CREATE},
    {QV_SW_SUB35_UNFUSED, "QVERSE_SUB35_UNFUSED", 0, 0, 1, QV_PARSE_ONE, QV_READ_AT_CREATE},
    {QV_SW_POST_GRAPH, "QVERSE_POST_GRAPH", 0, 0, 1, QV_PARSE_ATOI, QV_READ_ONCE},
    {QV_SW_CU_PARTITION, "QVERSE_CU_PARTITION", 0, 0, 1, QV_PARSE_ATOI, QV_READ_ONCE},
#ifdef QV_DEV_HOOKS
    {QV_SW_SKIP, "QVERSE_SKIP", 0, 0, 255, QV_PARSE_ATOI, QV_READ_ONCE},
    {QV_SW_DUP, "QVERSE_DUP", 0, 0, 255, QV_PARSE_ATOI, QV_READ_ONCE},
#endif
};

struct QvSwitches {
    int v[QV_SW_COUNT];
    int operator[](int id) const { return v[id]; }
    bool operator==(const QvSwitches &o) const {
        for (int i = 0; i < QV_SW_COUNT; ++i)
            if (v[i] != o.v[i]) return false;
        return true;
    }
    QvSwitches forward_part() const {
        QvSwitches f = *this;
        for (int id : {(int)QV_KV_SPANS, (int)QV_KV_FWD_GRAPH, (int)QV_KV_CTC, (int)QV_KV_RESERVED, (int)QV_SW_POST_GRAPH}) f.v[id] = 0;
        return f;
    }
};

inline void qv_switches_read_env(QvSwitches &e, QvWhen when) {
    for (const QvSwitchRow &r : QV_SWITCH_TABLE) {
        if (r.when != when) continue;
        const char *s = r.parse == QV_PARSE_NONE ? nullptr : getenv(r.env);
        e.v[r.id] = !s ? r.dflt
                    : r.parse == QV_PARSE_DIGIT ? (s[0] >= '0' && s[0] <= '9' ? atoi(s) : r.dflt)
                    : r.parse == QV_PARSE_ATOI ? atoi(s) : s[0] == '1';
    }
    if (when == QV_READ_ONCE)
        e.v[QV_SW_ATT] = e.v[QV_SW_ATT_OLD] ? 2 : e.v[QV_SW_ATT_HPB] ? 1 : e.v[QV_SW_ATT_TILED] ? 0 : e.v[QV_SW_ATT_X] ? 5 : QV_SWITCH_TABLE[QV_SW_ATT].dflt;
}

inline const QvSwitches &qv_switches_env() {
    static const QvSwitches env = [] {
        QvSwitches e;
        qv_switches_read_env(e, QV_READ_ONCE);
        qv_switches_read_env(e, QV_READ_AT_CREATE);
        return e;
    }();
    return env;
}

struct QvOverrides {
    std::atomic<int> v[QV_SW_COUNT];
    QvOverrides() { for (std::atomic<int> &a : v) a.store(-1); }
};
inline QvOverrides g_qv_overrides;

inline void qv_switch_set(int id, int mode) {
    if (id >= 0 && id < QV_SW_COUNT) g_qv_overrides.v[id].store(mode < 0 ? -1 : mode);
}
inline void qv_kernel_variant_set(int which, int mode) { if (which < QV_KV_COUNT) qv_switch_set(which, mode); }
inline void qv_attention_set_variant(int mode) { qv_switch_set(QV_SW_ATT, mode); }
inline void qv_gemm_set_t256(int mode) { qv_switch_set(QV_SW_GEMM_T256, mode); }
inline void qv_gemm_set_bm(int mode) { qv_switch_set(QV_SW_GEMM_BM, mode); }

inline QvSwitches qv_switches_now(bool creating = false) {
    QvSwitches sw = qv_switches_env();
    if (creating) qv_switches_read_env(sw, QV_READ_AT_CREATE);
    for (int i = 0; i < QV_SW_COUNT; ++i) {
        const int o = g_qv_overrides.v[i].load();
        if (o >= 0) sw.v[i] = o;
    }
    return sw;
}
```

offline-tarteel_amd/engine.py:

```python

from __future__ import annotations

import ctypes as C
import os
from pathlib import Path

import numpy as np

from . import LIB_PATH, TABLES_PATH
from .normalizer import normalize_arabic
from .tables import Tables

QV_SOURCE = {0: None, 1: "text", 2: "ctc"}
QV_MAX_TRANSCRIPT = 1024
QV_MAX_TRANSCRIPT_WIDE = 2048


def front_window(text: str, limit: int = QV_MAX_TRANSCRIPT) -> str:
    if len(text) <= limit:
        return text
    cut = text.rfind(" ", 0, limit + 1)
    return text[:cut] if cut > 0 else text[:limit]
FLAG_EMPTY, FLAG_TRUNC, FLAG_USED_CTC, FLAG_CAND_OVERFLOW = 1, 2, 4, 8

# ... 208 lines not shown
def load_library(path: Path | str | None = None) -> C.CDLL:
    global _lib
    if _lib is not None:
        return _lib
    p = Path(path or os.environ.get("QVERSE_LIB", LIB_PATH))
    if not p.exists():
        raise QvError(f"{p} not found: build it with `python offline-tarteel_amd/build.py` "
                      "(hipcc, gfx950). There is no CPU fallback for this path.")
    lib = C.CDLL(str(p))
    vp, i32, i64 = C.c_void_p, C.c_int32, C.c_int64
    lib.qv_config_default.argtypes = [C.POINTER(QvConfig)]
    lib.qv_config_default.restype = None
    lib.qv_create.argtypes = [C.POINTER(QvConfig), C.POINTER(vp)]
    lib.qv_destroy.argtypes = [vp]
    lib.qv_destroy.restype = None
    lib.qv_last_error.argtypes = [vp]
    lib.qv_last_error.restype = C.c_char_p
    lib.qv_build_info.restype = C.c_char_p
    lib.qv_frames_for_samples.argtypes = [i64]
    lib.qv_frames_for_samples.restype = i32
    lib.qv_forward.argtypes = [vp, vp, vp, i32, i64, vp, i32, vp, vp]
    lib.qv_decode_retrieve_rerank.argtypes = [vp, vp, vp, i32, i32, vp, vp, vp]
    lib.qv_decode_retrieve_rerank_async.argtypes = [vp, vp, vp, i32, i32, vp]
    lib.qv_fetch_results.argtypes = [vp, i32, i32, vp, vp, vp]
    lib.qv_predict_batch.argtypes = [vp, vp, vp, i32, i64, vp, vp, vp]
    lib.qv_predict_batch_async.argtypes = [vp, vp, vp, i32, i64, vp]
    lib.qv_predict_batch_async_ctx.argtypes = [vp, vp, vp, i32, i64, vp, vp]
    lib.qv_packed_results_dev.argtypes = [vp]
    lib.qv_packed_results_dev.restype = vp
    lib.qv_upfirdn.argtypes = [vp, vp, i64, vp, i32, i32, i32, i64, i64, vp, vp]
    lib.qv_upfirdn_batch.argtypes = [vp, vp, i64, vp, vp, i32, vp, i32, i32, i32, i64, vp, i64, vp]
    lib.qv_mixdown_batch.argtypes = [vp, vp, i64, vp, i32, i32, vp, i64, vp]
    lib.qv_context_count.argtypes = [vp]
    lib.qv_max_transcript.argtypes = [vp]
    lib.qv_max_transcript.restype = i32
    lib.qv_probe_concurrent_streams.argtypes = []
    lib.qv_last_context.argtypes = [vp]
    lib.qv_wait_ctx.argtypes = [vp, i32]
    lib.qv_packed_results_ctx.argtypes = [vp, i32, vp]
    lib.qv_packed_results_ctx.restype = vp
    lib.qv_fetch_results_ctx.argtypes = [vp, i32, i32, i32, vp, vp]
    lib.qv_align.argtypes = [vp, vp, vp, i32, i32, vp, vp, vp, vp, vp, vp, i32, vp]
    lib.qv_align_results_ctx.argtypes = [vp, i32, i32, vp, vp, vp, vp, vp, i32]
    lib.qv_nbest_results_ctx.argtypes = [vp, i32, i32, i32, i32, vp, vp]
    lib.qv_nbest_select.argtypes = [vp, vp, vp, vp, i32, i32, i32, vp, vp, vp]
    lib.qv_correct.argtypes = [vp, vp, vp, vp, vp, i32, i32, vp, vp, i32, vp, i32, vp]
    lib.qv_correct_results_ctx.argtypes = [vp, i32, i32, i32, vp, vp, i32, vp, i32]
    lib.qv_transcribe.argtypes = [vp, vp, vp, i32, i32, vp, vp, vp, vp, vp, i32, vp]
    lib.qv_transcribe_batch.argtypes = [vp, vp, vp, i32, i64, vp, vp, vp, vp, vp, i32, vp]
    lib.qv_long_plan.argtypes = [i64, i32, i32, i32, vp, vp, vp, vp]
    lib.qv_transcribe_long.argtypes = [vp, vp, i64, vp, i32, i32, i32, vp, vp, vp, vp, vp, i32, vp]
    lib.qv_transcribe_windows.argtypes = [vp, vp, i32, vp, i32, i32, i32, vp, vp, vp, vp, vp, i32, vp]
    lib.qv_long_kernel_times.argtypes = [vp, vp]
    lib.qv_align_long_plan.argtypes = [vp, vp, i32, i32, i32, i32, vp, vp]
    lib.qv_align_windows.argtypes = [vp, vp, i32, vp, i32, i32, i32, vp, vp, vp, vp, vp, vp, i32, vp]
    lib.qv_align_long.argtypes = [vp, vp, i64, vp, i32, i32, i32, vp, vp, vp, vp, vp, vp, i32, vp]
    lib.qv_align_long_kernel_times.argtypes = [vp, vp]
    lib.qv_trie_stats.argtypes = [C.c_char_p, i32, vp, vp, vp, vp]
    lib.qv_trie_node_tokens.argtypes = [vp, i32, i32, vp, i32, vp]
    lib.qv_beam_decode.argtypes = [vp, vp, vp, i32, i32, i32, i32, i32, vp, vp, vp, i32, vp]
    lib.qv_beam_batch.argtypes = [vp, vp, vp, i32, i64, i32, i32, i32, vp, vp, vp, i32, vp]
    lib.qv_scan_stats.argtypes = [C.c_char_p, i32, i32, vp, vp, vp, vp]
    lib.qv_scan_logprobs.argtypes = [vp, vp, vp, i32, i32, i32, C.c_double, i32, vp, vp, vp, vp, vp]
    lib.qv_scan_batch.argtypes = [vp, vp, vp, i32, i64, i32, C.c_double, i32, vp, vp, vp, vp, vp]
    lib.qv_scan_kernel_times.argtypes = [vp, vp]
    lib.qv_tracker_match.argtypes = [vp, vp, vp, vp, vp, i32, vp, vp]
    lib.qv_match_verse.argtypes = [vp, vp, i32, i32, vp, vp, i32, vp, vp, vp, vp]
    lib.qv_debug_retrieve.argtypes = [vp, vp, i32, vp, vp, vp, vp, vp, vp, i32, vp, vp, vp, vp, vp]
    lib.qv_debug_ctc_loss.argtypes = [vp, vp, i32, vp, vp, i32, vp, vp]
    lib.qv_debug_transcript_codes.argtypes = [vp, i32, i32, vp, i32, vp, vp]
    lib.qv_debug_forward_tap.argtypes = [vp, i32, i32, vp, vp]
    lib.qv_profile_gemm.argtypes = [vp, i32]
    lib.qv_profile_gemm_read.argtypes = [vp, vp, vp, vp]
    lib.qv_profile_replay_gemm.argtypes = [vp, i32, i32, vp, vp, vp]
    lib.qv_profile_replay_kernel.argtypes = [vp, i32, C.c_char_p, i32]
    lib.qv_debug_gemm_tiles.argtypes = [i32]
    lib.qv_debug_gemm_tile_height.argtypes = [i32]
    lib.qv_debug_gemm_pipeline.argtypes = [i32, i32, i32]
    lib.qv_debug_forward_graph_failures.argtypes = [vp]
    lib.qv_debug_forward_graph_failures.restype = i64
    lib.qv_debug_attention_variant.argtypes = [i32]
    lib.qv_debug_kernel_variant.argtypes = [i32, i32]
    lib.qv_debug_forward_graph_stats.argtypes = [vp, vp, vp]
    lib.qv_debug_sub01_plan.argtypes = [i64, i32, vp, vp]
    lib.qv_debug_sub35_plan.argtypes = [i64, i32, vp]
    lib.qv_weights_info.argtypes = [vp, C.c_char_p, i32]
    lib.qv_profile_inject_logprobs.argtypes = [vp, vp, i32, vp, i32]
    lib.qv_profile_stages.argtypes = [vp, i32]
    lib.qv_stage_times.argtypes = [vp, i32, vp]
    _lib = lib
    return lib


def exported_symbols() -> list[str]:
    import re

    hdr = (Path(__file__).resolve().parent.parent / "include" / "qverse.h").read_text()
    return sorted(set(re.findall(r"\b(qv_[a-z_0-9]+)\s*\(", hdr)))


def env_knobs() -> dict:
    return dict(
        top_text=int(os.getenv("CTC_DIRECT_TOP_TEXT", "100")),
        top_span_refs=int(os.getenv("CTC_DIRECT_TOP_SPAN_REFS", "80")),
        max_span=int(os.getenv("CTC_DIRECT_MAX_SPAN", "6")),
        threshold=float(os.getenv("CTC_DIRECT_THRESHOLD", "0.80")),
        text_weight=float(os.getenv("CTC_DIRECT_TEXT_WEIGHT", "0.0")),
        span_penalty=float(os.getenv("CTC_DIRECT_SPAN_PENALTY", "0.5")),
        stream_gate=stream_gate_default(),
    )


_long_env = None


def long_env() -> tuple[float | None, float | None]:
    global _long_env
    if _long_env is None:
        def num(name):
            v = os.environ.get(name, "").strip()
            return float(v) if v else None
        _long_env = (num("QVERSE_LONG_WINDOW_S"), num("QVERSE_LONG_MARGIN_S"))
    return _long_env


def stream_gate_default() -> bool:
    return os.getenv("QVERSE_STREAM_GATE", "0") == "1"


class Engine:

    def __init__(self, device: int = 0, with_model: bool = True, weights_path: str | None = None,
                 seed: int = 20260630, precision: int = 0, max_batch: int = 64, max_samples: int = 480000,
                 tables_path: str | None = None, skip_unused_passes: bool = True, contexts: int = 1,
                 max_transcript: int = QV_MAX_TRANSCRIPT, **knobs):
        import torch

        if not torch.cuda.is_available():
            raise QvError("no ROCm device visible: the qverse hot path runs on MI355X only (no CPU fallback)")
        self.torch = torch
        self.lib = load_library()
        self.device = device
        self.tables_path = str(tables_path or TABLES_PATH)
        if not Path(self.tables_path).exists():
            raise FileNotFoundError(self.tables_path)
        if weights_path is not None and not Path(weights_path).exists():
            raise FileNotFoundError(f"No weight file at {weights_path}")
        cfg = QvConfig()
        self.lib.qv_config_default(C.byref(cfg))
        cfg.device = device
        self._keep = (self.tables_path.encode(), weights_path.encode() if weights_path else None)
        cfg.tables_path, cfg.weights_path = self._keep
        cfg.random_weights_seed = seed
        cfg.with_model = int(with_model)
        cfg.precision = precision
        cfg.max_batch = max_batch
        cfg.max_samples = max_samples
        cfg.skip_unused_passes = int(skip_unused_passes)
        cfg.n_contexts = int(contexts)
        cfg.max_transcript = int(max_transcript)
        self.contexts = int(contexts)
        kn = env_knobs()
        kn.update(knobs)
        kn.pop("stream_gate", None)
        for k, v in kn.items():
            setattr(cfg, k, v)
# ... 302 lines not shown
        y = torch.empty(n_out, dtype=torch.float32, device=x.device)
        rc = self.lib.qv_upfirdn(self.h, C.c_void_p(x.data_ptr()), n_in, _p(taps), len(taps),
                                 up, down, m0, n_out, C.c_void_p(y.data_ptr()), self._stream())
        self._check(rc, "qv_upfirdn")
        return y

    RESAMPLE_ROWS = 1024

    def resample_rows(self, x, lengths, up: int, down: int, src_rows=None, out_pitch: int | None = None):
        from .audio import resample_plan

        torch = self.torch
        assert x.is_cuda and x.dtype == torch.float32 and x.dim() == 2 and x.stride(1) == 1
        lens = np.ascontiguousarray(np.asarray(lengths, dtype=np.int64))
        rows = len(lens)
        plan = [resample_plan(up, down, int(n)) for n in sorted(set(lens.tolist()))]
        up_r, down_r, m0 = plan[0][0], plan[0][1], plan[0][3]
        if up_r == down_r == 1:
            y = x if src_rows is None else x[torch.as_tensor(list(src_rows), device=x.device)]
            return y.clone(), lens.tolist()
        taps = max((p[2] for p in plan), key=len)
        n_out = [int((int(n) * up_r + down_r - 1) // down_r) for n in lens]
        pitch = int(out_pitch or max(n_out))
        assert pitch >= max(n_out)
        y = torch.empty((rows, pitch), dtype=torch.float32, device=x.device)
        src = None if src_rows is None else np.ascontiguousarray(np.asarray(list(src_rows), dtype=np.int32))
        x_pitch = int(x.stride(0))
        for r0 in range(0, rows, self.RESAMPLE_ROWS):
            r1 = min(rows, r0 + self.RESAMPLE_ROWS)
            ln_c = lens[r0:r1]
            src_c = None if src is None else src[r0:r1]
            x_ptr = x.data_ptr() + (0 if src is not None else r0 * x_pitch * 4)
            rc = self.lib.qv_upfirdn_batch(self.h, C.c_void_p(x_ptr), x_pitch, _p(src_c), _p(ln_c), r1 - r0, _p(taps), len(taps),
                                           up_r, down_r, m0, C.c_void_p(y.data_ptr() + r0 * pitch * 4), pitch, self._stream())
            self._check(rc, "qv_upfirdn_batch")
        return y, n_out

    def mixdown_rows(self, x, n_frames, channels: int):
        torch = self.torch
        assert x.is_cuda and x.dtype == torch.float32 and x.dim() == 2 and x.stride(1) == 1
        nf = np.ascontiguousarray(np.asarray(n_frames, dtype=np.int64))
        y = torch.zeros((len(nf), int(nf.max())), dtype=torch.float32, device=x.device)
        x_pitch, y_pitch = int(x.stride(0)), int(y.stride(0))
        for r0 in range(0, len(nf), self.RESAMPLE_ROWS):
            nf_c = nf[r0:r0 + self.RESAMPLE_ROWS]
            rc = self.lib.qv_mixdown_batch(self.h, C.c_void_p(x.data_ptr() + r0 * x_pitch * 4), x_pitch, _p(nf_c), len(nf_c), int(channels),
                                           C.c_void_p(y.data_ptr() + r0 * y_pitch * 4), y_pitch, self._stream())
            self._check(rc, "qv_mixdown_batch")
        return y

    def speed_perturb_rows(self, x, lengths, factor: float, src_rows=None):
        return self.resample_rows(x, lengths, int(factor * 10), 10, src_rows=src_rows)

    def speed_perturb(self, x, factor: float):
        return x if factor == 1.0 else self.resample_poly(x, int(factor * 10), 10)

    GEMM_EPILOGUES = ["f16", "f16_swish", "f16_relu", "glu", "resid", "f32", "qkv"]

    def gemm_tiles(self, mode: int):
        self._check(self.lib.qv_debug_gemm_tiles(int(mode)), "qv_debug_gemm_tiles")

    def gemm_tile_height(self, mode: int):
        self._check(self.lib.qv_debug_gemm_tile_height(int(mode)), "qv_debug_gemm_tile_height")

    def gemm_pipeline(self, ld: int = -1, nst: int = -1, narrow: int = -1):
        self._check(self.lib.qv_debug_gemm_pipeline(int(ld), int(nst), int(narrow)), "qv_debug_gemm_pipeline")

    def replay_kernel(self, which: int) -> str:
        name = C.create_string_buffer(64)
        self._check(self.lib.qv_profile_replay_kernel(self.h, which, name, 64), "qv_profile_replay_kernel")
        return name.value.decode()

    def weights_info(self) -> str:
        buf = C.create_string_buffer(512)
        self._check(self.lib.qv_weights_info(self.h, buf, 512), "qv_weights_info")
        return buf.value.decode()

    def attention_variant(self, mode: int):
        self._check(self.lib.qv_debug_attention_variant(int(mode)), "qv_debug_attention_variant")

    def kernel_variant(self, which: int, mode: int):
        self._check(self.lib.qv_debug_kernel_variant(int(which), int(mode)), "qv_debug_kernel_variant")

    def forward_graph_stats(self) -> dict:
        r, c = C.c_int64(0), C.c_int64(0)
        self._check(self.lib.qv_debug_forward_graph_stats(self.h, C.byref(r), C.byref(c)), "qv_debug_forward_graph_stats")
        return {"replays": int(r.value), "captures": int(c.value)}

    def profile_gemm(self, enable: bool):
        self._check(self.lib.qv_profile_gemm(self.h, int(enable)), "qv_profile_gemm")

    def profile_gemm_read(self) -> list[dict]:
        ms = np.zeros(21)
        fl = np.zeros(21)
        n = np.zeros(21, np.int32)
        self._check(self.lib.qv_profile_gemm_read(self.h, _p(ms), _p(fl), _p(n)), "qv_profile_gemm_read")
        out = []
        for c in range(21):
            if n[c]:
                epi, tile = self.GEMM_EPILOGUES[c // 3], c % 3
                out.append({"kernel": f"k_gemm256<{epi}>" if tile == 2 else f"k_gemm<{epi},{128 if tile else 64}>",
                            "ms": float(ms[c]), "flops": float(fl[c]), "launches": int(n[c])})
        return out

    def inject_logprobs(self, log_probs=None, t_frames=None):
        if log_probs is None:
            self._injected = None
            self._check(self.lib.qv_profile_inject_logprobs(self.h, None, 0, None, 0), "qv_profile_inject_logprobs")
            return
        B, t_max, t = self._logprob_args(log_probs, t_frames, per_row=False)
        self._injected = log_probs
        self._check(self.lib.qv_profile_inject_logprobs(self.h, C.c_void_p(log_probs.data_ptr()), t_max, _p(t), B), "qv_profile_inject_logprobs")

    def profile_stages(self, enable: bool):
        self._check(self.lib.qv_profile_stages(self.h, int(enable)), "qv_profile_stages")

    def stage_times(self, ctx: int | None = None) -> dict:
        if ctx is None:
            ctx = int(self.lib.qv_last_context(self.h))
        ms = np.zeros(4, np.float32)
        self._check(self.lib.qv_stage_times(self.h, ctx, _p(ms)), "qv_stage_times")
        return {k: float(v) * 1e-3 for k, v in zip(("forward", "decode", "build", "rerank"), ms)}

    REPLAY_SHAPES = ["FFN-up [M,512]x[512,2048]+Swish", "FFN-down [M,2048]x[2048,512]+residual", "QKV [M,512]x[512,1536]",
                     "attention out [M,512]x[512,512]+residual", "pointwise conv [M,512]x[512,1024]+GLU"]

    def replay_gemm(self, which: int, iters: int = 50) -> dict:
        us, fl = C.c_double(), C.c_double()
        self._check(self.lib.qv_profile_replay_gemm(self.h, which, iters, C.byref(us), C.byref(fl), self._stream()),
                    "qv_profile_replay_gemm")
        name = C.create_string_buffer(64)
        self._check(self.lib.qv_profile_replay_kernel(self.h, which, name, 64), "qv_profile_replay_kernel")
        return {"kernel": name.value.decode(), "shape": self.REPLAY_SHAPES[which], "avg_us": us.value,
                "flops": fl.value, "launches": iters}

    def next_verse(self, surah: int, ayah: int) -> int:
        t = self.tables.s
        if not (1 <= surah <= 114) or not (1 <= ayah <= int(t["surah_len"][surah - 1])):
            return -1
        idx = int(t["surah_start"][surah - 1]) + ayah - 1
        return idx + 1 if idx + 1 < self.tables.n_verses else -1

    def track_match(self, texts, last_refs=None) -> list[dict | None]:
        n = len(texts)
        if n == 0:
            return []
        last_refs = last_refs or [None] * n
        texts = [front_window(t, self.max_transcript) for t in texts]
        enc = [self.tables.encode(t) for t in texts]
        off = np.zeros(n + 1, np.int32)
        off[1:] = np.cumsum([len(e) for e in enc])
        codes = np.ascontiguousarray(np.concatenate(enc) if off[-1] else np.zeros(1, np.uint8))
        nw = np.ascontiguousarray(np.array([len(t.split()) for t in texts], np.int32))
        bonus = np.ascontiguousarray(np.array([self.next_verse(*r) if r else -1 for r in last_refs], np.int32))
        out = (QvTrackMatch * n)()
        rc = self.lib.qv_tracker_match(self.h, _p(codes), _p(off), _p(nw), _p(bonus), n, C.cast(out, C.c_void_p),
                                       self._stream())
        self._check(rc, "qv_tracker_match")
        return [None if m.verse < 0 else
                {"surah": m.surah, "ayah": m.ayah, "n_words": m.n_words, "score": m.score, "verse": m.verse,
                 "variant": m.variant} for m in out]

    def continuation_bonuses(self, hint) -> list[tuple[int, float]]:
        if not hint:
            return []
        s, a = hint
# ... 390 lines not shown
```

Measured before the change: 18450 utterances/s.

## Fuse CTC head GEMM with log-softmax and per-frame argmax

Adds a dedicated k_head_lsm kernel that computes the 512x1025 CTC head projection with MFMA for 32 rows per block. It applies bias and log-softmax in LDS, writes log-probs directly, and emits a per-frame argmax id. The greedy decode kernel then copies these precomputed ids instead of rescanning the full log-prob tensor, and the separate logits buffer and logsoftmax launch are skipped on the fp16 path. The trade-off is a large-LDS single-block-per-CU kernel that may underuse the GPU for small M, plus a new graph variant key for the post-processing chain.

```diff
diff --git a/include/qverse.h b/include/qverse.h
--- a/include/qverse.h
+++ b/include/qverse.h
@@ -309,6 +309,8 @@
 
 int qv_debug_kernel_variant(int32_t which, int32_t mode);
 
+int qv_debug_decode_paths(qv_engine *eng, int64_t *copies, int64_t *scans);
+
 int qv_debug_sub01_plan(int64_t n_samples, int32_t batch, int32_t *frames_out, int32_t *run_tiles_out);
 int qv_debug_sub35_plan(int64_t n_samples, int32_t batch, int32_t *run_frames_out);
 
diff --git a/offline-tarteel_amd/csrc/qv_capi.hip b/offline-tarteel_amd/csrc/qv_capi.hip
--- a/offline-tarteel_amd/csrc/qv_capi.hip
+++ b/offline-tarteel_amd/csrc/qv_capi.hip
@@ -526,7 +526,10 @@
         rc = qv_post_run(eng, c, eng->inject_lp, eng->inject_tmax, eng->inject_t.data(), batch, run);
         if (rc == QV_OK) align_note(c, eng->inject_lp, eng->inject_tmax, batch, run);
     } else {
-        rc = qv_post_run(eng, c, c.logprobs_ws, t_max, t_out.data(), batch, run);
+        const int16_t *frame_id = nullptr;
+        const int32_t *row_off = nullptr;
+        qv_model_frame_ids(eng->model, eng->cur_ctx, &frame_id, &row_off);
+        rc = qv_post_run(eng, c, c.logprobs_ws, t_max, t_out.data(), batch, run, frame_id, row_off);
         if (rc == QV_OK) align_note(c, c.logprobs_ws, t_max, batch, run);
     }
     if (rc) return rc;
@@ -1233,6 +1236,14 @@
     return QV_OK;
 }
 
+extern "C" int qv_debug_decode_paths(qv_engine *eng, int64_t *copies, int64_t *scans) {
+    QV_SERIALISE(eng);
+    if (!eng || !copies || !scans) return QV_ERR_ARG;
+    *copies = eng->decode_copies;
+    *scans = eng->decode_scans;
+    return QV_OK;
+}
+
 extern "C" int64_t qv_debug_forward_graph_failures(qv_engine *eng) {
     QV_SERIALISE(eng);
     return (eng && eng->model) ? qv_model_graph_failures(eng->model) : -1;
diff --git a/offline-tarteel_amd/csrc/qv_common.h b/offline-tarteel_amd/csrc/qv_common.h
--- a/offline-tarteel_amd/csrc/qv_common.h
+++ b/offline-tarteel_amd/csrc/qv_common.h
@@ -294,7 +294,7 @@
     int decode_threads;
     int frag_blocks;
     size_t trigram_lds;
-    void (*k_decode)(QvTables, QvWork, const float *, int, const int32_t *);
+    void (*k_decode)(QvTables, QvWork, const float *, int, const int32_t *, const int16_t *, const int32_t *);
     void (*k_prepare_codes)(QvWork, int);
     void (*k_trigram)(QvTables, QvWork), (*k_frag)(QvTables, QvWork);
     void (*k_lcs_full)(QvTables, QvWork, int), (*k_hint_sp)(QvTables, QvWork, int);
@@ -308,7 +308,7 @@
                           const int32_t *n_words_host, const int32_t *bonus_host, int batch,
                           qv_track_match *out_host, hipStream_t stream);
 int qv_post_run(qv_engine *eng, QvCtx &c, const float *logprobs_dev, int t_max, const int32_t *t_host, int batch,
-                hipStream_t stream);
+                hipStream_t stream, const int16_t *frame_id = nullptr, const int32_t *row_off = nullptr);
 int qv_post_debug_retrieve(qv_engine *eng, QvCtx &c, const uint8_t *codes_host, int n, hipStream_t stream);
 int qv_post_match_verse(qv_engine *eng, QvCtx &c, const uint8_t *codes_host, int n, int n_bonus, const int32_t *bonus_verse,
                         const double *bonus_value, int max_span, hipStream_t stream);
@@ -329,6 +329,7 @@
 
 void qv_model_weights_info(const QvModel *m, char *out, int cap);
 void qv_model_graph_stats(const QvModel *m, int64_t *replays, int64_t *captures);
+void qv_model_frame_ids(const QvModel *m, int k, const int16_t **frame_id, const int32_t **row_off);
 int64_t qv_model_graph_failures(const QvModel *m);
 void qv_stage_mark(qv_engine *eng, QvCtx &c, int i, hipStream_t s);
 
@@ -390,6 +391,7 @@
     QvScanState *scan = nullptr;
     bool profile_stages;
     const float *inject_lp;
+    int64_t decode_copies = 0, decode_scans = 0;
     int inject_tmax, inject_batch;
     std::vector<int32_t> inject_t;
     std::vector<uint8_t> h_surah;
diff --git a/offline-tarteel_amd/csrc/qv_dev_util.h b/offline-tarteel_amd/csrc/qv_dev_util.h
--- a/offline-tarteel_amd/csrc/qv_dev_util.h
+++ b/offline-tarteel_amd/csrc/qv_dev_util.h
@@ -16,6 +16,23 @@
 #pragma unroll
     for (int o = 32; o > 0; o >>= 1) v = fminf(v, __shfl_xor(v, o));
     return v;
+}
+
+static __device__ __forceinline__ void logsoftmax_row(const float *p, int lane, float v[17]) {
+    float mx = -INFINITY;
+#pragma unroll
+    for (int i = 0; i < 17; ++i) {
+        int c = lane + 64 * i;
+        v[i] = c < 1025 ? p[c] : -INFINITY;
+        mx = fmaxf(mx, v[i]);
+    }
+    mx = wave_max(mx);
+    float s = 0.f;
+#pragma unroll
+    for (int i = 0; i < 17; ++i) s += (lane + 64 * i < 1025) ? expf(v[i] - mx) : 0.f;
+    float lse = mx + logf(wave_sum(s));
+#pragma unroll
+    for (int i = 0; i < 17; ++i) v[i] = v[i] - lse;
 }
 
 static __device__ __forceinline__ int xcd_order(int wg, int nwg) {
diff --git a/offline-tarteel_amd/csrc/qv_head.hip b/offline-tarteel_amd/csrc/qv_head.hip
--- /dev/null
+++ b/offline-tarteel_amd/csrc/qv_head.hip
@@ -0,0 +1,128 @@
+#include "qv_layers.h"
+#include "qv_dev_util.h"
+#include "qv_gemm_epilogue.h"
+#include "qv_greedy.h"
+#include "qv_launch_plan.h"
+
+namespace {
+
+typedef unsigned int u32x4_t __attribute__((ext_vector_type(4)));
+
+#define HEAD_NF 4
+static_assert(HEAD_NF * 8 * 32 + 1 == QV_VOCAB && HEAD_ROWS == 32 && QV_D == 512, "k_head_lsm is built for 32 rows x 1025 columns x 512");
+
+__global__ __launch_bounds__(512, 1) void k_head_lsm(const half_t *__restrict__ xh, const half_t *__restrict__ W,
+                                                     const float *__restrict__ bias, float *__restrict__ out,
+                                                     int16_t *__restrict__ frame_id, int M, const int32_t *__restrict__ row_map,
+                                                     int t_out) {
+    extern __shared__ __attribute__((aligned(256))) unsigned char s_head[];
+    const int tid = threadIdx.x, lane = tid & 63, wave = tid >> 6, l31 = lane & 31, hi = lane >> 5;
+    const int m0 = xcd_order(blockIdx.x, gridDim.x) * HEAD_ROWS;
+
+    const __amdgpu_buffer_rsrc_t rsA = __builtin_amdgcn_make_buffer_rsrc((void *)xh, 0, M * (QV_D * 2), 0x00020000);
+    u32x4_t ra[4];
+#pragma unroll
+    for (int p = 0; p < 4; ++p) {
+        const int ci = tid + 512 * p, row = ci >> 6, cc = ci & 63;
+        ra[p] = __builtin_amdgcn_raw_buffer_load_b128(rsA, ((m0 + row) * QV_D + cc * 8) * 2, 0, 0);
+    }
+    const half_t *wp[HEAD_NF];
+#pragma unroll
+    for (int j = 0; j < HEAD_NF; ++j) wp[j] = W + (size_t)((wave + 8 * j) * 32 + l31) * QV_D + hi * 8;
+    half8 wb[2][HEAD_NF][4];
+    auto fetch = [&](int kt, half8 (&w)[HEAD_NF][4]) {
+#pragma unroll
+        for (int j = 0; j < HEAD_NF; ++j)
+#pragma unroll
+            for (int s = 0; s < 4; ++s) w[j][s] = *(const half8 *)(wp[j] + kt * 64 + s * 16);
+    };
+    fetch(0, wb[0]);
+#pragma unroll
+    for (int p = 0; p < 4; ++p) {
+        const int ci = tid + 512 * p, row = ci >> 6, kt = (ci & 63) >> 3, c = ci & 7;
+        *(u32x4_t *)(s_head + kt * (HEAD_ROWS * 128) + row * 128 + ((c ^ ((row >> 1) & 7)) << 4)) = ra[p];
+    }
+    __syncthreads();
+    auto a_frag = [&](int ks) {
+        const int c = (ks & 3) * 2 + hi;
+        return *(const half8 *)(s_head + (ks >> 2) * (HEAD_ROWS * 128) + l31 * 128 + ((c ^ ((l31 >> 1) & 7)) << 4));
+    };
+
+    f32x16 acc[HEAD_NF];
+#pragma unroll
+    for (int j = 0; j < HEAD_NF; ++j)
+#pragma unroll
+        for (int r = 0; r < 16; ++r) acc[j][r] = 0.f;
+#pragma unroll
+    for (int kt = 0; kt < QV_D / 64; ++kt) {
+        if (kt + 1 < QV_D / 64) fetch(kt + 1, wb[(kt + 1) & 1]);
+#pragma unroll
+        for (int s = 0; s < 4; ++s) {
+            const half8 af = a_frag(kt * 4 + s);
+#pragma unroll
+            for (int j = 0; j < HEAD_NF; ++j) acc[j] = __builtin_amdgcn_mfma_f32_32x32x16_f16(wb[kt & 1][j][s], af, acc[j], 0, 0, 0);
+        }
+    }
+    f32x16 acc_t;
+    if (wave == 0) {
+        half8 wt[QV_D / 16];
+#pragma unroll
+        for (int ks = 0; ks < QV_D / 16; ++ks) wt[ks] = *(const half8 *)(W + (size_t)(1024 + l31) * QV_D + ks * 16 + hi * 8);
+#pragma unroll
+        for (int r = 0; r < 16; ++r) acc_t[r] = 0.f;
+#pragma unroll
+        for (int ks = 0; ks < QV_D / 16; ++ks) acc_t = __builtin_amdgcn_mfma_f32_32x32x16_f16(wt[ks], a_frag(ks), acc_t, 0, 0, 0);
+    }
+    __syncthreads();
+
+    float *const sL = (float *)s_head;
+#pragma unroll
+    for (int j = 0; j < HEAD_NF; ++j)
+#pragma unroll
+        for (int q = 0; q < 4; ++q) {
+            const int col = (wave + 8 * j) * 32 + 8 * q + 4 * hi;
+            const f32x4 bb = *(const f32x4 *)(bias + col);
+            f32x4 v;
+#pragma unroll
+            for (int e = 0; e < 4; ++e) v[e] = qv_epi::val_f32<false>(acc[j][q * 4 + e], 1.f, 1.f, bb[e]);
+            *(f32x4 *)(sL + l31 * HEAD_PITCH + col) = v;
+        }
+    if (wave == 0 && hi == 0) sL[l31 * HEAD_PITCH + 1024] = qv_epi::val_f32<false>(acc_t[0], 1.f, 1.f, bias[1024]);
+    __syncthreads();
+
+    for (int r = wave; r < HEAD_ROWS && m0 + r < M; r += 8) {
+        const int row = m0 + r;
+        const int bt = row_map[row];
+        const size_t orow = (size_t)(bt >> 16) * t_out + (bt & 0xFFFF);
+        float *p = sL + r * HEAD_PITCH;
+        float v[17];
+        logsoftmax_row(p, lane, v);
+        float *o = out + orow * 1025;
+#pragma unroll
+        for (int i = 0; i < 17; ++i) {
+            int c = lane + 64 * i;
+            if (c < 1025) { o[c] = v[i]; p[c] = v[i]; }
+        }
+        float best;
+        int bi;
+        frame_argmax(p, lane, best, bi);
+        if (lane == 0) frame_id[row] = (int16_t)bi;
+    }
+}
+
+}
+
+void qv_head_init() {
+    static const int once = [] {
+        (void)hipFuncSetAttribute((const void *)k_head_lsm, hipFuncAttributeMaxDynamicSharedMemorySize, HEAD_LDS);
+        return 0;
+    }();
+    (void)once;
+}
+
+void launch_head_lsm(const half_t *xh, const half_t *w, const float *bias, float *out, int16_t *frame_id, int M,
+                     const int32_t *row_map, int t_out, hipStream_t s) {
+    qv_head_init();
+    hipLaunchKernelGGL(k_head_lsm, dim3((M + HEAD_ROWS - 1) / HEAD_ROWS), dim3(512), HEAD_LDS, s, xh, w, bias, out, frame_id, M, row_map,
+                       t_out);
+}
diff --git a/offline-tarteel_amd/csrc/qv_launch_plan.h b/offline-tarteel_amd/csrc/qv_launch_plan.h
--- a/offline-tarteel_amd/csrc/qv_launch_plan.h
+++ b/offline-tarteel_amd/csrc/qv_launch_plan.h
@@ -98,3 +98,23 @@
     p.rest = variant == 4 || variant == 5 ? ATT_X_192 : variant == 1 ? ATT_WS_1_3_256 : ATT_WS_2_2_192;
     return p;
 }
+
+#define HEAD_ROWS 32
+#define HEAD_PITCH 1028
+#define HEAD_LDS (HEAD_ROWS * HEAD_PITCH * 4)
+static_assert(HEAD_PITCH >= QV_VOCAB && HEAD_PITCH % 32 == 4 && HEAD_LDS >= HEAD_ROWS * 512 * 2 && HEAD_LDS <= 160 * 1024,
+              "k_head_lsm: one block per CU, 160 KB of LDS");
+struct HeadPlan {
+    bool fused;
+    int blocks;
+    int lds_bytes;
+    bool ids_valid;
+};
+inline HeadPlan head_plan(int M, int precision, bool taps, bool gemm_prof, const QvSwitches &sw) {
+    HeadPlan p;
+    p.fused = sw[QV_KV_HEAD] == 0 && precision != 2 && !taps && !gemm_prof;
+    p.blocks = p.fused ? (M + HEAD_ROWS - 1) / HEAD_ROWS : (M + 3) / 4;
+    p.lds_bytes = p.fused ? HEAD_LDS : 0;
+    p.ids_valid = p.fused;
+    return p;
+}
diff --git a/offline-tarteel_amd/csrc/qv_layers.h b/offline-tarteel_amd/csrc/qv_layers.h
--- a/offline-tarteel_amd/csrc/qv_layers.h
+++ b/offline-tarteel_amd/csrc/qv_layers.h
@@ -43,6 +43,9 @@
 void launch_dwconv1d(const half_t *x, const float *w, const float *bias, const int32_t *len, const int32_t *row_off, half_t *y,
                      int t_max, int batch, hipStream_t s);
 void launch_logsoftmax(const float *logits, int ld, float *out, int M, const int32_t *row_map, int t_out, hipStream_t s);
+void launch_head_lsm(const half_t *xh, const half_t *w, const float *bias, float *out, int16_t *frame_id, int M,
+                     const int32_t *row_map, int t_out, hipStream_t s);
+void qv_head_init();
 void launch_zero_pad_rows(float *out, const int32_t *len, int t_out, int t_min, int batch, hipStream_t s);
 void launch_upfirdn_rows(const float *x, int64_t x_pitch, const int32_t *src, const int64_t *n_in_rows, int rows, const float *hflip,
                          int P, int up, int down, int64_t m0, float *y, int64_t y_pitch, hipStream_t s);
diff --git a/offline-tarteel_amd/csrc/qv_layers.hip b/offline-tarteel_amd/csrc/qv_layers.hip
--- a/offline-tarteel_amd/csrc/qv_layers.hip
+++ b/offline-tarteel_amd/csrc/qv_layers.hip
@@ -766,25 +766,13 @@
     if (row >= M) return;
     const int bt = row_map[row];
     const size_t orow = (size_t)(bt >> 16) * t_out + (bt & 0xFFFF);
-    const float *p = logits + (size_t)row * ld;
     float v[17];
-    float mx = -INFINITY;
+    logsoftmax_row(logits + (size_t)row * ld, lane, v);
+    float *o = out + orow * 1025;
 #pragma unroll
     for (int i = 0; i < 17; ++i) {
         int c = lane + 64 * i;
-        v[i] = c < 1025 ? p[c] : -INFINITY;
-        mx = fmaxf(mx, v[i]);
-    }
-    mx = wave_max(mx);
-    float s = 0.f;
-#pragma unroll
-    for (int i = 0; i < 17; ++i) s += (lane + 64 * i < 1025) ? expf(v[i] - mx) : 0.f;
-    float lse = mx + logf(wave_sum(s));
-    float *o = out + orow * 1025;
-#pragma unroll
-    for (int i = 0; i < 17; ++i) {
-        int c = lane + 64 * i;
-        if (c < 1025) o[c] = v[i] - lse;
+        if (c < 1025) o[c] = v[i];
     }
 }
 
diff --git a/offline-tarteel_amd/csrc/qv_match_body.inc b/offline-tarteel_amd/csrc/qv_match_body.inc
--- a/offline-tarteel_amd/csrc/qv_match_body.inc
+++ b/offline-tarteel_amd/csrc/qv_match_body.inc
@@ -8,7 +8,8 @@
 
 #define DEC_WAVES 16
 __global__ __launch_bounds__(64 * DEC_WAVES) void k_decode(QvTables tab, QvWork wk, const float *__restrict__ lp, int t_max,
-                                                          const int32_t *__restrict__ t_dev) {
+                                                          const int32_t *__restrict__ t_dev, const int16_t *__restrict__ frame_id,
+                                                          const int32_t *__restrict__ row_off) {
     __shared__ uint8_t raw[QV_RAW_CAP];
     __shared__ unsigned long long pm[2][QV_NSYM][QV_MAXW];
     __shared__ int16_t s_fid[QV_FRAME_CAP];
@@ -17,11 +18,16 @@
     if (b == 0 && tid == 0) { *wk.n_fail = 0; wk.frag_ctr[0] = 0; wk.frag_ctr[1] = 0; wk.frag_ctr[2] = 0; }
     QvUtt &u = wk.utt[b];
     const int T = t_dev[b];
-    for (int t = wave; t < T; t += DEC_WAVES) {
-        float best;
-        int bi;
-        frame_argmax(lp + ((size_t)b * t_max + t) * QV_VOCAB, lane, best, bi);
-        if (lane == 0) s_fid[t] = (int16_t)bi;
+    if (frame_id) {
+        const int16_t *ids = frame_id + row_off[b];
+        for (int t = tid; t < T; t += 64 * DEC_WAVES) s_fid[t] = ids[t];
+    } else {
+        for (int t = wave; t < T; t += DEC_WAVES) {
+            float best;
+            int bi;
+            frame_argmax(lp + ((size_t)b * t_max + t) * QV_VOCAB, lane, best, bi);
+            if (lane == 0) s_fid[t] = (int16_t)bi;
+        }
     }
     __syncthreads();
     if (wave != 0) return;
diff --git a/offline-tarteel_amd/csrc/qv_model.hip b/offline-tarteel_amd/csrc/qv_model.hip
--- a/offline-tarteel_amd/csrc/qv_model.hip
+++ b/offline-tarteel_amd/csrc/qv_model.hip
@@ -1,6 +1,7 @@
 
 #include "qv_common.h"
 #include "qv_graph.h"
+#include "qv_launch_plan.h"
 #include "qv_layers.h"
 #include "qv_ort.h"
 #include "qv_model_prep_host.h"
@@ -79,6 +80,8 @@
     int lens_slot = 0, lens_last = 0;
     float *tap_x;
     FwdShape last = {};
+    int16_t *frame_id = nullptr;
+    bool ids_valid = false;
     bool sub35 = false;
     float *c1f, *c1pf, *c2f, *gluf, *dwf;
     int8_t *q8;
@@ -179,7 +182,9 @@
     TRY(qv_dev_zeroed(eng, m->allocs, M * QV_D, &a.glu));
     TRY(qv_dev_zeroed(eng, m->allocs, M * QV_D, &a.dw));
     TRY(qv_dev_zeroed(eng, m->allocs, M * QV_D, &a.xh));
-    TRY(qv_dev_zeroed(eng, m->allocs, M * HEAD_N, &a.logits));
+    a.logits = nullptr;
+    if (m->ort || m->save_taps) TRY(qv_dev_zeroed(eng, m->allocs, M * HEAD_N, &a.logits));
+    if (!m->ort) TRY(qv_dev_zeroed(eng, m->allocs, M, &a.frame_id));
     TRY(qv_dev_zeroed(eng, m->allocs, lens_words, &a.lens_dev));
     TRY(qv_dev_zeroed(eng, m->allocs, M, &a.row_map));
     QV_HIP(hipHostMalloc((void **)&a.lens_host, sizeof(int32_t) * lens_words * QV_STAGE_SLOTS, hipHostMallocDefault));
@@ -252,6 +257,7 @@
     m->save_taps = sw[QV_SW_DEBUG_TAPS] != 0;
     m->n_ctx = eng->n_ctx;
     qv_sub35_init();
+    qv_head_init();
     for (int k = 0; k < m->n_ctx; ++k) TRY(alloc_context(eng, m, k, sw[QV_SW_SUB_UNFUSED] != 0, sw[QV_SW_SUB35_UNFUSED] != 0));
     return QV_OK;
 }
@@ -435,8 +441,10 @@
         }, false);
         return save_x(l + 1);
     }
-    void ctc_head() const {
-        if (m->ort) {
+    void ctc_head(const HeadPlan &head, float *logprobs) const {
+        if (head.fused) {
+            launch_head_lsm(a.xh, m->w.head_w, m->w.head_b, logprobs, a.frame_id, sh.M, a.row_map, sh.t_max_out, s);
+        } else if (m->ort) {
             const RowOwner own = {a.row_map, nullptr, 0, 0};
             launch_rows_minmax(a.x, sh.M, a.row_map, mm(MM_HEAD), s);
             launch_quant_rows(a.x, sh.M, QV_D, own, mm(MM_HEAD), a.q8, s);
@@ -448,7 +456,7 @@
 };
 
 int launch_all(qv_engine *eng, const QvModel *m, const QvActs &a, const FwdShape &sh, const float *audio, int64_t n_max, float *logprobs,
-               const half_t *posp, const QvSwitches &sw, hipStream_t s) {
+               const half_t *posp, const QvSwitches &sw, const HeadPlan &head, hipStream_t s) {
     const Fwd f = {eng, m, a, sh, dev_lens(m, a), audio, n_max, posp, sw, s};
     if (m->ort) f.frontend_ort();
     else if (!(hook_skip() & 32)) f.frontend_f16();
@@ -467,8 +475,8 @@
         TRY(f.layer_out(l));
     }
     if (hook_skip() & 2) launch_to_half(a.x, a.xh, (size_t)sh.M * QV_D, s);
-    f.ctc_head();
-    launch_logsoftmax(a.logits, HEAD_N, logprobs, sh.M, a.row_map, sh.t_max_out, s);
+    f.ctc_head(head, logprobs);
+    if (!head.fused) launch_logsoftmax(a.logits, HEAD_N, logprobs, sh.M, a.row_map, sh.t_max_out, s);
     if (sh.t_min_pad >= 0) launch_zero_pad_rows(logprobs, f.d.l3, sh.t_max_out, sh.t_min_pad, sh.B, s);
     return QV_OK;
 }
@@ -487,7 +495,10 @@
     const QvSwitches sw = qv_switches_now();
     const half_t *posp = nullptr;
     TRY(get_pos(eng, m, sh.T, sw, s, &posp));
-    auto plain = [&] { return launch_all(eng, m, a, sh, audio, n_max, logprobs, posp, sw, s); };
+    const HeadPlan head = head_plan(sh.M, m->ort ? QV_PREC_ORT_MIXED : m->w4 ? QV_PREC_MIXED_INT4_INT8 : QV_PREC_FP16, m->save_taps,
+                                    qv_gemm_prof_on(), sw);
+    if (!head.fused && !a.logits) TRY(qv_dev_zeroed(eng, m->allocs, m->rows_cap * HEAD_N, &a.logits));
+    auto plain = [&] { return launch_all(eng, m, a, sh, audio, n_max, logprobs, posp, sw, head, s); };
     FwdGraphs &graphs = a.fwd_graphs;
     FwdGraphs::Plan plan = {graphs.PLAIN, -1, false};
     if (sw[QV_KV_FWD_GRAPH] == 1 && may_graph && !m->save_taps && !eng->profile_stages && !qv_gemm_prof_on()) {
@@ -516,7 +527,14 @@
     else TRY(plain());
     QV_HIP(hipGetLastError());
     a.last = sh;
-    return QV_OK;
+    a.ids_valid = head.ids_valid;
+    return QV_OK;
+}
+
+void qv_model_frame_ids(const QvModel *m, int k, const int16_t **frame_id, const int32_t **row_off) {
+    const QvActs &a = m->ctx_acts[k];
+    *frame_id = a.ids_valid ? a.frame_id : nullptr;
+    *row_off = a.ids_valid ? dev_lens(m, a).row_off : nullptr;
 }
 
 static int replay_args(qv_engine *eng, QvModel *m, int k, int which, GemmArgs &g, int &epi) {
diff --git a/offline-tarteel_amd/csrc/qv_postlogits.hip b/offline-tarteel_amd/csrc/qv_postlogits.hip
--- a/offline-tarteel_amd/csrc/qv_postlogits.hip
+++ b/offline-tarteel_amd/csrc/qv_postlogits.hip
@@ -478,7 +478,8 @@
     hipLaunchKernelGGL(k, dim3(batch, 64), dim3(256), 0, stream, tab, wk, kn, lp, t_max);
 }
 
-int qv_post_run(qv_engine *eng, QvCtx &c, const float *lp, int t_max, const int32_t *t_host, int batch, hipStream_t stream) {
+int qv_post_run(qv_engine *eng, QvCtx &c, const float *lp, int t_max, const int32_t *t_host, int batch, hipStream_t stream,
+                const int16_t *frame_id, const int32_t *row_off) {
     const QvSwitches sw = qv_switches_now();
     const QvMatchSet &set = *eng->match;
     QvTables &tab = eng->tab;
@@ -506,7 +507,7 @@
 #endif
     auto launch_chain = [&]() -> int {
         if (skip & 128) return QV_OK;
-        hipLaunchKernelGGL(set.k_decode, dim3(batch), dim3(set.decode_threads), 0, stream, tab, wk, lp, t_max, c.t_dev);
+        hipLaunchKernelGGL(set.k_decode, dim3(batch), dim3(set.decode_threads), 0, stream, tab, wk, lp, t_max, c.t_dev, frame_id, row_off);
         qv_stage_mark(eng, c, 2, stream);
         launch_retrieval(eng, c, batch, 0, stream, sw);
         qv_stage_mark(eng, c, 3, stream);
@@ -517,7 +518,7 @@
     };
     QvCtx::PostGraph *hit = nullptr;
     if (sw[QV_SW_POST_GRAPH] != 0 && !c.post_graph_off && eng->n_ctx > 1 && stream == c.stream && lp == c.logprobs_ws && !eng->profile_stages) {
-        const int variants = sw[QV_KV_SPANS] | (sw[QV_KV_CTC] << 4) | ((set.max_q > QV_MAX_TRANSCRIPT) << 8);
+        const int variants = sw[QV_KV_SPANS] | (sw[QV_KV_CTC] << 4) | ((set.max_q > QV_MAX_TRANSCRIPT) << 8) | ((frame_id != nullptr) << 9);
         for (int i = 0; i < c.n_post_graph; ++i)
             if (c.post_graph[i].lp == lp && c.post_graph[i].batch == batch && c.post_graph[i].t_max == t_max && c.post_graph[i].variants == variants)
                 hit = &c.post_graph[i];
@@ -538,6 +539,7 @@
         if (rc) return rc;
     }
     QV_HIP(hipGetLastError());
+    if (!(skip & 128)) ++(frame_id ? eng->decode_copies : eng->decode_scans);
     c.last_batch = batch;
     c.last_tmax = t_max;
     return QV_OK;
diff --git a/offline-tarteel_amd/csrc/qv_switches.h b/offline-tarteel_amd/csrc/qv_switches.h
--- a/offline-tarteel_amd/csrc/qv_switches.h
+++ b/offline-tarteel_amd/csrc/qv_switches.h
@@ -7,7 +7,7 @@
 
 enum {
     QV_KV_LOGMEL = 0, QV_KV_ORT_SUB = 1, QV_KV_SPANS = 2, QV_KV_FWD_GRAPH = 3, QV_KV_CTC = 4, QV_KV_SUB_RUN = 5, QV_KV_SUB35 = 6,
-    QV_KV_RESERVED = 7, QV_KV_COUNT = 8,
+    QV_KV_HEAD = 7, QV_KV_COUNT = 8,
     QV_SW_ATT = 8, QV_SW_ATT_OLD, QV_SW_ATT_HPB, QV_SW_ATT_TILED, QV_SW_ATT_X,
     QV_SW_GEMM_T256, QV_SW_GEMM_BM, QV_SW_GEMM_NST, QV_SW_GEMM_NARROW, QV_SW_GEMM_LD, QV_SW_GEMM_MINTILES, QV_SW_GEMM_MINTILES_LONGK,
     QV_SW_DEBUG_TAPS, QV_SW_SUB_UNFUSED, QV_SW_SUB35_UNFUSED, QV_SW_POST_GRAPH, QV_SW_CU_PARTITION,
@@ -36,7 +36,7 @@
     {QV_KV_CTC, "QVERSE_CTC", 1, 0, 15, QV_PARSE_DIGIT, QV_READ_ONCE},
     {QV_KV_SUB_RUN, "QVERSE_SUB_RUN", 0, 0, 15, QV_PARSE_DIGIT, QV_READ_ONCE},
     {QV_KV_SUB35, nullptr, 0, 0, 15, QV_PARSE_NONE, QV_READ_ONCE},
-    {QV_KV_RESERVED, nullptr, 0, 0, 15, QV_PARSE_NONE, QV_READ_ONCE},
+    {QV_KV_HEAD, nullptr, 0, 0, 15, QV_PARSE_NONE, QV_READ_ONCE},
     {QV_SW_ATT, nullptr, 3, 0, 5, QV_PARSE_NONE, QV_READ_ONCE},
     {QV_SW_ATT_OLD, "QVERSE_ATT_OLD", 0, 0, 1, QV_PARSE_ONE, QV_READ_ONCE},
     {QV_SW_ATT_HPB, "QVERSE_ATT_HPB", 0, 0, 1, QV_PARSE_ONE, QV_READ_ONCE},
@@ -70,7 +70,7 @@
     }
     QvSwitches forward_part() const {
         QvSwitches f = *this;
-        for (int id : {(int)QV_KV_SPANS, (int)QV_KV_FWD_GRAPH, (int)QV_KV_CTC, (int)QV_KV_RESERVED, (int)QV_SW_POST_GRAPH}) f.v[id] = 0;
+        for (int id : {(int)QV_KV_SPANS, (int)QV_KV_FWD_GRAPH, (int)QV_KV_CTC, (int)QV_SW_POST_GRAPH}) f.v[id] = 0;
         return f;
     }
 };
diff --git a/offline-tarteel_amd/engine.py b/offline-tarteel_amd/engine.py
--- a/offline-tarteel_amd/engine.py
+++ b/offline-tarteel_amd/engine.py
@@ -314,6 +314,7 @@
     lib.qv_debug_attention_variant.argtypes = [i32]
     lib.qv_debug_kernel_variant.argtypes = [i32, i32]
     lib.qv_debug_forward_graph_stats.argtypes = [vp, vp, vp]
+    lib.qv_debug_decode_paths.argtypes = [vp, vp, vp]
     lib.qv_debug_sub01_plan.argtypes = [i64, i32, vp, vp]
     lib.qv_debug_sub35_plan.argtypes = [i64, i32, vp]
     lib.qv_weights_info.argtypes = [vp, C.c_char_p, i32]
@@ -782,6 +783,11 @@
     def kernel_variant(self, which: int, mode: int):
         self._check(self.lib.qv_debug_kernel_variant(int(which), int(mode)), "qv_debug_kernel_variant")
 
+    def decode_paths(self) -> dict:
+        c, s = C.c_int64(0), C.c_int64(0)
+        self._check(self.lib.qv_debug_decode_paths(self.h, C.byref(c), C.byref(s)), "qv_debug_decode_paths")
+        return {"copies": int(c.value), "scans": int(s.value)}
+
     def forward_graph_stats(self) -> dict:
         r, c = C.c_int64(0), C.c_int64(0)
         self._check(self.lib.qv_debug_forward_graph_stats(self.h, C.byref(r), C.byref(c)), "qv_debug_forward_graph_stats")
```

Result: no change. 18300 utterances/s (-0.8%).
